# Anaesthesiaye/sound_event_detection_transformer

Measured on AMD Instinct MI355X. Metric: audio clips/sec training throughput (B=64, 10s@64-mel), higher is better.
Workload: dtype bf16; 1 GPU; URBAN-SED SEDT enc_layers=3 dec_at num_queries=10 B=64/GPU, 10 s @ 64-mel (B,1,500,64), full train step: fwd + Hungarian matching (device) + SetCriterion + bwd + clip 0.1 + AdamW, dropout 0.1; global_batch=64, parallelism=dp1

## Files before the change

sound_event_detection_transformer_amd/csrc/misc.hip:

```cpp
#include <stdarg.h>
#include <string.h>
#include <type_traits>
#include <algorithm>
#include "common.h"

namespace sedt {

static thread_local char g_err[512] = "";

void set_error(const char* fmt, ...) {
  va_list ap;
  va_start(ap, fmt);
  vsnprintf(g_err, sizeof(g_err), fmt, ap);
  va_end(ap);
}

int check_launch(const char* what) {
  hipError_t e = hipGetLastError();
  if (e != hipSuccess) {
    set_error("%s: launch failed: %s", what, hipGetErrorString(e));
    return 2;
  }
  return 0;
}

static inline hipStream_t S(void* s) { return reinterpret_cast<hipStream_t>(s); }
static inline unsigned nblk(long n, int per = 256) { return (unsigned)((n + per - 1) / per); }


struct ReduceJobs {
  int n;
  SedtReduceJob j[SEDT_MAX_REDUCE_JOBS];
  const uint32_t* pf[3]; int pf_lines[3];
};

__host__ __device__ inline int reduce_job_mode(const SedtReduceJob& J) {
  if ((reinterpret_cast<uintptr_t>(J.slab) | reinterpret_cast<uintptr_t>(J.out)) & 15) return 2;
  if (J.taps == 1 && (J.Ci & 3) == 0) return J.splitk >= 16 ? 3 : 0;
  if (J.taps > 1 && J.taps <= 9 && (J.Ci & 63) == 0) return 1;
  return 2;
}
__host__ __device__ inline int reduce_job_blocks(const SedtReduceJob& J) {
  const long per = (long)J.R * J.taps * J.Ci;
  const int mode = reduce_job_mode(J);
  if (mode == 0) return (int)((per + 1023) / 1024);
  if (mode == 1) return J.R * (J.Ci / 64);
  return (int)((per + 255) / 256);
}

__global__ __launch_bounds__(256) void multi_wgrad_reduce_kernel(const ReduceJobs jobs) {
  __shared__ float tile[9][65];
  if (blockIdx.x < 256 && jobs.pf_lines[0] + jobs.pf_lines[1] + jobs.pf_lines[2] > 0) {
    const int slot = blockIdx.x >> 3, nslots = min(32, max(1, (int)(gridDim.x >> 3)));
    uint32_t acc = 0;
    for (int r = 0; r < 3; ++r)
      for (int j = slot * 256 + threadIdx.x; j < jobs.pf_lines[r]; j += nslots * 256) acc ^= jobs.pf[r][(long)j * 32];
    if (acc == 0x9e3779b9u && jobs.n < 0) tile[0][0] = 1.f;
  }
  int lo = 0, hi = jobs.n - 1;
  while (lo < hi) {
    int mid = (lo + hi + 1) >> 1;
    if (jobs.j[mid].blk0 <= (int)blockIdx.x) lo = mid; else hi = mid - 1;
  }
  const SedtReduceJob& J = jobs.j[lo];
  const int blk = blockIdx.x - J.blk0;
  const long per = (long)J.R * J.taps * J.Ci;
  if (J.colsum_slab) {
    __shared__ float csum[4][64];
    const int col = blk * 64 + (threadIdx.x & 63), zg = threadIdx.x >> 6;
    if (blk * 64 < J.R) {
      float b0 = 0.f, b1 = 0.f, b2 = 0.f, b3 = 0.f;
      if (col < J.R) {
        const float* cp = J.colsum_slab + col;
        const int csk = J.cs_splitk > 0 ? J.cs_splitk : J.splitk;
        int z = zg;
        for (; z + 12 < csk; z += 16) {
          b0 += cp[(long)z * J.R];
          b1 += cp[(long)(z + 4) * J.R];
          b2 += cp[(long)(z + 8) * J.R];
          b3 += cp[(long)(z + 12) * J.R];
        }
        for (; z < csk; z += 4) b0 += cp[(long)z * J.R];
      }
      csum[zg][threadIdx.x & 63] = (b0 + b1) + (b2 + b3);
      __syncthreads();
      if (zg == 0 && col < J.R) J.bias_out[col] = (csum[0][col & 63] + csum[1][col & 63]) + (csum[2][col & 63] + csum[3][col & 63]);
    }
  }
  const int mode = reduce_job_mode(J);
  if (mode == 3) {
    __shared__ float4 zsum[4][64];
    const int q = threadIdx.x & 63, zg = threadIdx.x >> 6;
    const long e = ((long)blk * 64 + q) * 4;
    float4 s0 = make_float4(0.f, 0.f, 0.f, 0.f), s1 = s0;
    if (e < per) {
      const float* sp = J.slab + e;
      int z = zg;
      for (; z + 4 < J.splitk; z += 8) {
        const float4 a = *reinterpret_cast<const float4*>(sp + (long)z * per);
        const float4 b = *reinterpret_cast<const float4*>(sp + (long)(z + 4) * per);
        s0.x += a.x; s0.y += a.y; s0.z += a.z; s0.w += a.w;
        s1.x += b.x; s1.y += b.y; s1.z += b.z; s1.w += b.w;
      }
      if (z < J.splitk) {
        const float4 a = *reinterpret_cast<const float4*>(sp + (long)z * per);
        s0.x += a.x; s0.y += a.y; s0.z += a.z; s0.w += a.w;
      }
    }
    zsum[zg][q] = make_float4(s0.x + s1.x, s0.y + s1.y, s0.z + s1.z, s0.w + s1.w);
    __syncthreads();
    if (zg == 0 && e < per) {
      const float4 a = zsum[0][q], b = zsum[1][q], c = zsum[2][q], d = zsum[3][q];
      float4 s = make_float4((a.x + b.x) + (c.x + d.x), (a.y + b.y) + (c.y + d.y), (a.z + b.z) + (c.z + d.z), (a.w + b.w) + (c.w + d.w));
      if (J.rowscale) {
        const float sc = J.rowscale[e / J.Ci];
        s.x *= sc; s.y *= sc; s.z *= sc; s.w *= sc;
      }
      *reinterpret_cast<float4*>(J.out + e) = s;
    }
  } else if (mode == 0) {
    const long e = ((long)blk * 256 + threadIdx.x) * 4;
    if (e >= per) return;
    const float* sp = J.slab + e;
    float4 s0 = *reinterpret_cast<const float4*>(sp), s1 = make_float4(0.f, 0.f, 0.f, 0.f), s2 = s1, s3 = s1;
    int z = 1;
    for (; z + 4 <= J.splitk; z += 4) {
      const float4 a = *reinterpret_cast<const float4*>(sp + (long)z * per);
      const float4 b = *reinterpret_cast<const float4*>(sp + (long)(z + 1) * per);
      const float4 c = *reinterpret_cast<const float4*>(sp + (long)(z + 2) * per);
      const float4 d = *reinterpret_cast<const float4*>(sp + (long)(z + 3) * per);
      s0.x += a.x; s0.y += a.y; s0.z += a.z; s0.w += a.w;
      s1.x += b.x; s1.y += b.y; s1.z += b.z; s1.w += b.w;
      s2.x += c.x; s2.y += c.y; s2.z += c.z; s2.w += c.w;
      s3.x += d.x; s3.y += d.y; s3.z += d.z; s3.w += d.w;
    }
    for (; z < J.splitk; ++z) {
      const float4 a = *reinterpret_cast<const float4*>(sp + (long)z * per);
      s0.x += a.x; s0.y += a.y; s0.z += a.z; s0.w += a.w;
    }
    float4 s = make_float4((s0.x + s1.x) + (s2.x + s3.x), (s0.y + s1.y) + (s2.y + s3.y), (s0.z + s1.z) + (s2.z + s3.z),
                           (s0.w + s1.w) + (s2.w + s3.w));
    if (J.rowscale) {
      const float sc = J.rowscale[e / J.Ci];
      s.x *= sc; s.y *= sc; s.z *= sc; s.w *= sc;
    }
    *reinterpret_cast<float4*>(J.out + e) = s;
  } else if (mode == 1) {
    const int chunks = J.Ci / 64;
    const int r = blk / chunks, c0 = (blk - r * chunks) * 64;
    if (r >= J.R) return;
    const int n = J.taps * 64;
    const float sc = J.rowscale ? J.rowscale[r] : 1.f;
    const long rbase = (long)r * J.taps * J.Ci;
    for (int i = threadIdx.x; i < n / 4; i += 256) {
      const int tap = i >> 4, c = (i & 15) * 4;
      const float* sp = J.slab + rbase + (long)tap * J.Ci + c0 + c;
      float4 v = *reinterpret_cast<const float4*>(sp), u = make_float4(0.f, 0.f, 0.f, 0.f);
      int z = 1;
      for (; z + 2 <= J.splitk; z += 2) {
        const float4 a = *reinterpret_cast<const float4*>(sp + (long)z * per);
        const float4 b = *reinterpret_cast<const float4*>(sp + (long)(z + 1) * per);
        v.x += a.x; v.y += a.y; v.z += a.z; v.w += a.w;
        u.x += b.x; u.y += b.y; u.z += b.z; u.w += b.w;
      }
      if (z < J.splitk) {
        const float4 a = *reinterpret_cast<const float4*>(sp + (long)z * per);
        v.x += a.x; v.y += a.y; v.z += a.z; v.w += a.w;
      }
      tile[tap][c] = (v.x + u.x) * sc; tile[tap][c + 1] = (v.y + u.y) * sc;
      tile[tap][c + 2] = (v.z + u.z) * sc; tile[tap][c + 3] = (v.w + u.w) * sc;
    }
    __syncthreads();
    float* o = J.out + ((long)r * J.Ci + c0) * J.taps;
    if (J.taps == 9) {
      for (int i = threadIdx.x; i < n / 4; i += 256) {
        float4 q;
        { const int k = 4 * i, c = k / 9, tap = k - c * 9; q.x = tile[tap][c]; }
        { const int k = 4 * i + 1, c = k / 9, tap = k - c * 9; q.y = tile[tap][c]; }
        { const int k = 4 * i + 2, c = k / 9, tap = k - c * 9; q.z = tile[tap][c]; }
        { const int k = 4 * i + 3, c = k / 9, tap = k - c * 9; q.w = tile[tap][c]; }
        *reinterpret_cast<float4*>(o + 4 * i) = q;
      }
    } else {
      for (int i = threadIdx.x; i < n; i += 256) {
        const int c = i / J.taps, tap = i - c * J.taps;
        o[i] = tile[tap][c];
      }
    }
  } else {
    const long e = (long)blk * 256 + threadIdx.x;
    if (e >= per) return;
    const int c = (int)(e % J.Ci);
    const long rt = e / J.Ci;
    const int tap = (int)(rt % J.taps);
    const int r = (int)(rt / J.taps);
    float s = 0.f;
    for (int z = 0; z < J.splitk; ++z) s += J.slab[(long)z * per + e];
    if (J.rowscale) s *= J.rowscale[r];
    J.out[((long)r * J.Ci + c) * J.taps + tap] = s;
  }
}

template <typename TI>
__global__ void colsum_kernel(const TI* __restrict__ in, long ld, int rows, int cols, int rows_per_chunk,
                              float* __restrict__ out) {
  __shared__ float red[4][64];
  int tx = threadIdx.x & 63, ty = threadIdx.x >> 6;
  int col = blockIdx.x * 64 + tx;
  int r0 = blockIdx.y * rows_per_chunk, r1 = min(rows, r0 + rows_per_chunk);
  float s = 0.f;
  if (col < cols)
    for (int r = r0 + ty; r < r1; r += 4) s += (float)in[(long)r * ld + col];
  red[ty][tx] = s;
  __syncthreads();
  if (ty == 0 && col < cols) out[(long)blockIdx.y * cols + col] = red[0][tx] + red[1][tx] + red[2][tx] + red[3][tx];
}

static int colsum_chunks(int rows) {
  int c = (rows + 255) / 256;
  return c < 1 ? 1 : (c > 256 ? 256 : c);
}

template <typename T>
__global__ void dropout_grad_kernel(const T* __restrict__ in, long ldi, T* __restrict__ out, long ldo, int rows, int cols,
                                    uint32_t thresh, float inv_keep, uint32_t seed, const uint32_t* seed_ptr) {
  long e = (long)blockIdx.x * blockDim.x + threadIdx.x;
  if (e >= (long)rows * cols) return;
  int r = (int)(e / cols), c = (int)(e % cols);
  uint32_t sd = eff_seed(seed, seed_ptr);
  float v = (float)in[(long)r * ldi + c];
  out[(long)r * ldo + c] = (T)(drop_keep(sd, (uint64_t)e, thresh) ? v * inv_keep : 0.f);
}

template <typename T>
__global__ void add_kernel(const T* __restrict__ a, const T* __restrict__ b, T* __restrict__ out, int rows, int cols,
                           int b_mod) {
  long e = (long)blockIdx.x * blockDim.x + threadIdx.x;
  if (e >= (long)rows * cols) return;
  int r = (int)(e / cols), c = (int)(e % cols);
  int rb = b_mod > 0 ? r % b_mod : r;
  out[e] = (T)((float)a[e] + (float)b[(long)rb * cols + c]);
}

struct AddN { const void* p[8]; int n; };
template <typename T>
__global__ void add_n_kernel(const AddN a, T* __restrict__ out, long n8) {
  const long e = (long)blockIdx.x * blockDim.x + threadIdx.x;
  if (e >= n8) return;
  float acc[8];
#pragma unroll
  for (int i = 0; i < 8; ++i) acc[i] = 0.f;
  for (int j = 0; j < a.n; ++j) {
    const VecT<T, 8> v = reinterpret_cast<const VecT<T, 8>*>(a.p[j])[e];
#pragma unroll
    for (int i = 0; i < 8; ++i) acc[i] += (float)v.v[i];
  }
  VecT<T, 8> o;
#pragma unroll
  for (int i = 0; i < 8; ++i) o.v[i] = (T)acc[i];
  reinterpret_cast<VecT<T, 8>*>(out)[e] = o;
}

template <typename TI, typename TO>
__global__ void cast_kernel(const TI* __restrict__ in, TO* __restrict__ out, long n) {
  long e = (long)blockIdx.x * blockDim.x + threadIdx.x;
  if (e < n) out[e] = (TO)(float)in[e];
}

template <typename T>
__global__ void relu_mask_kernel(const T* __restrict__ g, const T* __restrict__ y, T* __restrict__ out, long n) {
  long e = (long)blockIdx.x * blockDim.x + threadIdx.x;
  if (e < n) out[e] = ((float)y[e] > 0.f) ? g[e] : (T)0.f;
}

template <typename T>
__global__ void gelu_fwd_kernel(const T* __restrict__ h, T* __restrict__ a, long n8, uint32_t thresh, float inv_keep, uint32_t seed,
                                const uint32_t* seed_ptr) {
  const long e = (long)blockIdx.x * blockDim.x + threadIdx.x;
  if (e >= n8) return;
  const uint32_t sd = eff_seed(seed, seed_ptr);
  const VecT<T, 8> v = reinterpret_cast<const VecT<T, 8>*>(h)[e];
  VecT<T, 8> o;
#pragma unroll
  for (int i = 0; i < 8; ++i) {
    const float x = (float)v.v[i];
    const float y = 0.5f * x * (1.f + erff(x * 0.70710678118654752f));
    o.v[i] = (T)((thresh == 0u || drop_keep(sd, (uint64_t)(e * 8 + i), thresh)) ? y * inv_keep : 0.f);
  }
  reinterpret_cast<VecT<T, 8>*>(a)[e] = o;
}

template <typename T>
__global__ void gelu_bwd_kernel(const T* __restrict__ g, const T* __restrict__ h, T* __restrict__ out, long n8, uint32_t thresh,
                                float inv_keep, uint32_t seed, const uint32_t* seed_ptr) {
  const long e = (long)blockIdx.x * blockDim.x + threadIdx.x;
  if (e >= n8) return;
  const uint32_t sd = eff_seed(seed, seed_ptr);
  const VecT<T, 8> gv = reinterpret_cast<const VecT<T, 8>*>(g)[e];
  const VecT<T, 8> hv = reinterpret_cast<const VecT<T, 8>*>(h)[e];
  VecT<T, 8> o;
#pragma unroll
  for (int i = 0; i < 8; ++i) {
    const float x = (float)hv.v[i];
    const float d = 0.5f * (1.f + erff(x * 0.70710678118654752f)) + x * 0.39894228040143268f * expf(-0.5f * x * x);
    o.v[i] = (T)((thresh == 0u || drop_keep(sd, (uint64_t)(e * 8 + i), thresh)) ? (float)gv.v[i] * d * inv_keep : 0.f);
  }
  reinterpret_cast<VecT<T, 8>*>(out)[e] = o;
}

__global__ void sigmoid_grad_kernel(const float* g, const float* s, float* out, long n) {
  long e = (long)blockIdx.x * blockDim.x + threadIdx.x;
  if (e < n) out[e] = g[e] * s[e] * (1.f - s[e]);
}

constexpr int COPY_MAXJ = 8;
struct CopyJobs {
  int n;
  SedtCopyJob j[COPY_MAXJ];
};
__global__ __launch_bounds__(256) void copy2d_kernel(const CopyJobs jobs) {
  int i = 0;
  while (i + 1 < jobs.n && (int)blockIdx.x >= jobs.j[i + 1].blk0) ++i;
  const SedtCopyJob& J = jobs.j[i];
  const long w = (long)(blockIdx.x - J.blk0) * 256 + threadIdx.x;
  const long per = J.inner / 4;
  if (w >= per * J.outer) return;
  const long o = w / per, k = w - o * per;
  reinterpret_cast<uint32_t*>(reinterpret_cast<char*>(J.dst) + o * J.dst_stride)[k] =
      reinterpret_cast<const uint32_t*>(reinterpret_cast<const char*>(J.src) + o * J.src_stride)[k];
}

template <typename T>
__global__ void spsedt_dec_in_kernel(const T* __restrict__ patch, const float* __restrict__ query, const float* __restrict__ keep_in,
                                     float* __restrict__ keep_out, T* __restrict__ out, int B, int Q, int P, int qpp, int D, int train,
                                     uint32_t thresh, uint32_t seed, const uint32_t* seed_ptr) {
  const int row = blockIdx.x * (blockDim.x / 32) + threadIdx.x / 32;
  if (row >= B * Q) return;
  const int b = row / Q, q = row - b * Q, c0 = (threadIdx.x & 31) * 8;
  float k = 1.f;
  if (train) {
    if (keep_in) k = keep_in[(long)q * B + b];
    else k = (thresh == 0u || drop_keep(eff_seed(seed, seed_ptr), (uint64_t)q * B + b, thresh)) ? 1.f : 0.f;
    if (keep_out && c0 == 0) keep_out[(long)q * B + b] = k;
  }
  const float qs = train ? 2.f : 1.f;
  for (int c = c0; c < D; c += 256) {
    const VecT<T, 8> pv = *reinterpret_cast<const VecT<T, 8>*>(patch + ((long)b * P + q / qpp) * D + c);
    const float4 qa = *reinterpret_cast<const float4*>(query + (long)q * D + c), qb = *reinterpret_cast<const float4*>(query + (long)q * D + c + 4);
    const float qv[8] = {qa.x, qa.y, qa.z, qa.w, qb.x, qb.y, qb.z, qb.w};
    VecT<T, 8> o;
#pragma unroll
    for (int i = 0; i < 8; ++i) o.v[i] = (T)(qs * qv[i] + k * (float)pv.v[i]);
    *reinterpret_cast<VecT<T, 8>*>(out + (long)row * D + c) = o;
  }
}

template <typename T>
__global__ void spsedt_dec_in_bwd_kernel(const T* __restrict__ g, const float* __restrict__ keep, T* __restrict__ d_patch,
                                         float* __restrict__ d_query, int B, int Q, int P, int qpp, int D, int train) {
  __shared__ float part[3][1024 / 4];
  const int blk = blockIdx.x;
  const int c = threadIdx.x % D, grp = threadIdx.x / D;
  if (blk < B * P) {
    if (!d_patch || grp) return;
    const int b = blk / P, p = blk - b * P;
    float acc = 0.f;
    for (int r = 0; r < qpp; ++r) {
      const int q = p * qpp + r;
      if (q >= Q) break;
      const float k = (train && keep) ? keep[(long)q * B + b] : 1.f;
      acc += k * (float)g[((long)b * Q + q) * D + c];
    }
    d_patch[(long)blk * D + c] = (T)acc;
    return;
  }
  const int q = blk - B * P;
  const int per = (B + 3) / 4, b0 = grp * per, b1 = min(B, b0 + per);
  float acc = 0.f;
  int b = b0;
  for (; b + 8 <= b1; b += 8) {
    float v[8];
#pragma unroll
    for (int i = 0; i < 8; ++i) v[i] = (float)g[((long)(b + i) * Q + q) * D + c];
#pragma unroll
    for (int i = 0; i < 8; ++i) acc += v[i];
  }
  for (; b < b1; ++b) acc += (float)g[((long)b * Q + q) * D + c];
  if (grp) part[grp - 1][c] = acc;
  __syncthreads();
  if (!grp) d_query[(long)q * D + c] = (train ? 2.f : 1.f) * (((acc + part[0][c]) + part[1][c]) + part[2][c]);
}

__global__ void bn_fold_kernel(const float* w, const float* b, const float* rm, const float* rv, float* scale,
                               float* bias, int n) {
  int i = blockIdx.x * blockDim.x + threadIdx.x;
  if (i >= n) return;
  float sc = w[i] * rsqrtf(rv[i] + 1e-5f);
  scale[i] = sc;
  bias[i] = b[i] - rm[i] * sc;
}

template <typename T>
__global__ void pack_conv_kernel(const float* __restrict__ w, int Cout, int Cin, int taps, const float* bnscale,
                                 T* __restrict__ wf, T* __restrict__ wb) {
  long e = (long)blockIdx.x * blockDim.x + threadIdx.x;
  long n = (long)Cout * Cin * taps;
  if (e >= n) return;
  int tap = (int)(e % taps);
  long r = e / taps;
  int ci = (int)(r % Cin), co = (int)(r / Cin);
  float v = w[e];
  if (wf) wf[((long)co * taps + tap) * Cin + ci] = (T)v;
  if (wb) wb[((long)ci * taps + tap) * Cout + co] = (T)(bnscale ? v * bnscale[co] : v);
}

template <typename T>
__global__ void stem_prep_kernel(const float* w0, const float* b0, const float* w1, T* wcat) {
  int e = blockIdx.x * blockDim.x + threadIdx.x;
  if (e >= 64 * 128) return;
  int co = e >> 7, k = e & 127;
  float v = 0.f;
  int tap = k & 63;
  if (tap < 49) {
    const float* src = (k < 64) ? w0 : b0;
    for (int c = 0; c < 3; ++c) v += w1[(co * 3 + c) * 49 + tap] * src[c];
  }
  wcat[e] = (T)v;
}

template <typename T>
__global__ __launch_bounds__(256) void stem_im2col_kernel(const float* __restrict__ x, T* __restrict__ col, int B, int H, int W,
                                                          int Ho, int Wo) {
  extern __shared__ float rows[];
  const int P = W + 6;
  const int ho = blockIdx.y, b = blockIdx.z;
  const float* xb = x + (long)b * H * W;
  for (int i = threadIdx.x; i < 7 * P; i += 256) {
    const int kh = i / P, j = i - kh * P;
    const int hi = 2 * ho - 3 + kh, wi = j - 3;
    rows[i] = ((unsigned)hi < (unsigned)H && (unsigned)wi < (unsigned)W) ? xb[hi * W + wi] : 0.f;
  }
  __syncthreads();
  const int wo = blockIdx.x * 16 + (threadIdx.x >> 4), chunk = threadIdx.x & 15;
  if (wo >= Wo) return;
  const int pix = (b * Ho + ho) * Wo + wo;
  const int k0 = chunk * 8;
  const bool ind = k0 >= 64;
  VecT<T, 8> out;
#pragma unroll
  for (int e = 0; e < 8; ++e) {
    const int tap = (k0 & 63) + e;
    float v = 0.f;
    if (tap < 49) {
      const int kh = tap / 7, kw = tap - kh * 7;
      const int hi = 2 * ho - 3 + kh, wi = 2 * wo - 3 + kw;
      if (ind) v = ((unsigned)hi < (unsigned)H && (unsigned)wi < (unsigned)W) ? 1.f : 0.f;
      else v = rows[kh * P + 2 * wo + kw];
    }
    out.v[e] = (T)v;
  }
  *reinterpret_cast<VecT<T, 8>*>(col + (long)pix * 128 + k0) = out;
}

__global__ void stem_conv0_grad_kernel(const float* G, const float* w1, float* dw0, float* db0) {
  __shared__ float red[6][256];
  int t = threadIdx.x;
  float acc[6] = {0, 0, 0, 0, 0, 0};
  for (int e = t; e < 64 * 49; e += 256) {
    int co = e / 49, tap = e - co * 49;
    float gx = G[co * 128 + tap], gb = G[co * 128 + 64 + tap];
    for (int c = 0; c < 3; ++c) {
      float w = w1[(co * 3 + c) * 49 + tap];
      acc[c] += w * gx;
      acc[3 + c] += w * gb;
    }
  }
  for (int i = 0; i < 6; ++i) red[i][t] = acc[i];
  __syncthreads();
  for (int s = 128; s > 0; s >>= 1) {
    if (t < s)
      for (int i = 0; i < 6; ++i) red[i][t] += red[i][t + s];
    __syncthreads();
  }
  if (t < 3) dw0[t] = red[t][0];
  else if (t < 6) db0[t - 3] = red[t][0];
}

template <typename T, int VEC>
__global__ __launch_bounds__(256) void maxpool_fwd_kernel(const T* __restrict__ x, T* __restrict__ y, uint8_t* __restrict__ idx,
// ... 970 lines not shown
```

sound_event_detection_transformer_amd/functional.py:

```python
from collections import namedtuple

import torch
from torch.autograd import Function

from . import ops, packing, runtime
from .lib import F32, BF16
from .ops import ACT_NONE, ACT_RELU, ACT_SIGMOID, ConvGeom


def _dt_of(t):
    return F32 if t.dtype == torch.float32 else BF16


def _as(t, dt):
    want = torch.float32 if dt == F32 else torch.bfloat16
    t = t.contiguous()
    return t if t.dtype == want else ops.cast(t, dt)


def _wf(dt, w):
    return w if dt == F32 else ops.cast(w, BF16)


def _wb(dt, w):
    return ops.pack_conv(dt, w, want_fwd=False)[1]


def _prep_linear(dt, w, need_b):
    hit = packing.lookup(w)
    if hit is not None:
        return hit[0], hit[1]
    return _wf(dt, w), (_wb(dt, w) if need_b else None)


def _prep_conv(dt, w, bn):
    hit = packing.lookup(w)
    if hit is not None and hit[2] is not None:
        return hit
    sc, bi = ops.bn_fold(bn[0], bn[1], bn[2], bn[3])
    wf, wb = ops.pack_conv(dt, w, bnscale=sc)
    return wf, wb, sc, bi


class LinearFn(Function):

    @staticmethod
    def forward(ctx, x, weight, bias, act, out_f32, dt, relu_input=False, x_bits=None):
        x = _as(x, dt)
        ctx.relu_input = relu_input
        ctx.x_bits = x_bits if relu_input else None
        ctx.dt, ctx.act, ctx.out_f32 = dt, act, out_f32
        ctx.has_bias = bias is not None
        ctx.skinny = ops.skinny_ok(weight.shape[0], weight.shape[1]) and out_f32 and weight.is_contiguous()
        if ctx.skinny:
            y = ops.skinny_linear_fwd(dt, x, weight, bias, act, True)
            ctx.save_for_backward(x, weight, y if act != ACT_NONE else None)
            return y
        wf, ctx.wb = _prep_linear(dt, weight, ctx.needs_input_grad[0])
        y = ops.linear(dt, x, wf, bias=bias, act=act, out_f32=out_f32)
        ctx.save_for_backward(x, weight, y if act != ACT_NONE else None)
        return y

    @staticmethod
    def backward(ctx, gy):
        x, weight, y = ctx.saved_tensors
        dt = ctx.dt
        gy = gy.contiguous()
        if ctx.skinny:
            gx, gw, gb = ops.skinny_linear_bwd(dt, gy.float() if gy.dtype != torch.float32 else gy, y, weight, x, ctx.act,
                                               mask=x if ctx.relu_input else None, need_gx=ctx.needs_input_grad[0],
                                               need_gw=ctx.needs_input_grad[1], need_gb=ctx.has_bias and ctx.needs_input_grad[2])
            return gx, gw, gb, None, None, None, None, None
        if ctx.act == ACT_SIGMOID:
            gy = ops.sigmoid_grad(gy.float() if gy.dtype != torch.float32 else gy, y.float() if y.dtype != torch.float32 else y)
        elif ctx.act == ACT_RELU:
            gy = ops.relu_mask(_dt_of(gy), gy, y)
        g = _as(gy, dt)
        gx = None
        if ctx.needs_input_grad[0]:
            if ctx.relu_input and ctx.x_bits is not None:
                gx = ops.linear(dt, g, ctx.wb, mask=ctx.x_bits, ldm=ctx.x_bits.stride(0), mask_bits=True)
            else:
                gx = ops.linear(dt, g, ctx.wb, mask=x, ldm=x.stride(0)) if ctx.relu_input else ops.linear(dt, g, ctx.wb)
        gb = torch.empty((g.shape[1],), device=g.device, dtype=torch.float32) if (ctx.has_bias and ctx.needs_input_grad[2]) else None
        if ctx.needs_input_grad[1]:
            gw = ops.linear_wgrad(dt, g, x, bias_out=gb)
        else:
            gw = None
            if gb is not None:
                ops.colsum(dt, g, out=gb)
        return gx, gw, gb, None, None, None, None, None


class PoolAtFn(Function):

    @staticmethod
    def forward(ctx, logits, boxes, attn, mode, q0, Q):
        f32c = lambda t: t.detach() if (t.dtype == torch.float32 and t.is_contiguous()) else t.detach().float().contiguous()
        lg = f32c(logits)
        bx = f32c(boxes) if mode == 'weighted_sum' else None
        at = f32c(attn) if mode == 'attn' else None
        ctx.cfg = (mode, q0, Q)
        ctx.dts = (logits.dtype, None if boxes is None else boxes.dtype, None if attn is None else attn.dtype)
        ctx.save_for_backward(lg, bx, at)
        return ops.pool_at(lg, bx, at, mode, q0, Q)

    @staticmethod
    def backward(ctx, g):
        lg, bx, at = ctx.saved_tensors
        mode, q0, Q = ctx.cfg
        gl, gb, ga = ops.pool_at_bwd(lg, bx, at, mode, q0, Q, g)
        return (gl.to(ctx.dts[0]), None if gb is None else gb.to(ctx.dts[1]), None if ga is None else ga.to(ctx.dts[2]),
                None, None, None)


class HeadsFn(Function):

    @staticmethod
    def forward(ctx, hs, wc, bc, w1, b1, w2, b2, w3, b3, wa, ba, dt):
        Lh, B, Qp, d = hs.shape
        x = _as(hs, dt).view(Lh * B * Qp, d)
        tr = any(ctx.needs_input_grad)
        ctx.slab = None
        if ops.heads_slab_ok(dt, d, wc.shape[0], 0 if wa is None else wa.shape[0], hs.numel() // d) and wc.is_contiguous() and w3.is_contiguous():
            fr = [packing.lookup_frag(w) for w in (w1, w2)]
            if all(f is not None for f in fr):
                cls, box, at, hh = ops.heads_fwd(x, wc, bc, fr[0][0], b1, fr[1][0], b2, w3, b3, wa, ba, Lh, B, Qp, train=tr)
                ctx.dt, ctx.dims, ctx.has_at = dt, (Lh, B, Qp, d), wa is not None
                if tr:
                    ctx.slab = (fr[0][1], fr[1][1])
                    ctx.save_for_backward(x, hh[0], hh[1], box, at, wc, w3, wa)
                cls, box = cls.view(Lh, B, Qp, -1), box.view(Lh, B, Qp, 2)
                return (cls, box, at) if at is not None else (cls, box)
        cls = ops.skinny_linear_fwd(dt, x, wc, bc, ACT_NONE, True)
        w1f, w1b = _prep_linear(dt, w1, tr)
        w2f, w2b = _prep_linear(dt, w2, tr)
        h1 = ops.linear(dt, x, w1f, bias=b1, act=ACT_RELU)
        h2 = ops.linear(dt, h1, w2f, bias=b2, act=ACT_RELU)
        box = ops.skinny_linear_fwd(dt, h2, w3, b3, ACT_SIGMOID, True)
        at = None
        if wa is not None:
            xa = x.view(Lh, B, Qp, d)[Lh - 1, :, 0, :]
            at = ops.skinny_linear_fwd(dt, xa, wa, ba, ACT_SIGMOID, True)
        ctx.dt, ctx.dims, ctx.wb = dt, (Lh, B, Qp, d), (w1b, w2b)
        ctx.has_at = wa is not None
        ctx.save_for_backward(x, h1, h2, box, at, wc, w3, wa)
        cls, box = cls.view(Lh, B, Qp, -1), box.view(Lh, B, Qp, 2)
        return (cls, box, at) if at is not None else (cls, box)

    @staticmethod
    def backward(ctx, g_cls, g_box, g_at=None):
        x, h1, h2, box, at, wc, w3, wa = ctx.saved_tensors
        dt = ctx.dt
        Lh, B, Qp, d = ctx.dims
        M = Lh * B * Qp
        if ctx.slab is not None:
            f32c = lambda t: None if t is None else (t.contiguous() if t.dtype == torch.float32 else t.contiguous().float())
            C1, CA = wc.shape[0], 0 if wa is None else wa.shape[0]
            w1t, w2t = ctx.slab
            dhs, g_h1, g_h2, part = ops.heads_bwd(x, h1, h2, box.view(M, 2), at, f32c(g_cls).view(M, -1), f32c(g_box).view(M, 2),
                                                  f32c(g_at) if ctx.has_at else None, wc, w3, wa, w2t, w1t, Lh, B, Qp)
            rb = ops.ReduceBatch()
            d_b2 = torch.empty((d,), device=x.device, dtype=torch.float32)
            d_w2 = ops.linear_wgrad(dt, g_h2, h1, bias_out=d_b2, batch=rb)
            d_b1 = torch.empty((d,), device=x.device, dtype=torch.float32)
            d_w1 = ops.linear_wgrad(dt, g_h1, x, bias_out=d_b1, batch=rb)
            NG = C1 + CA + 2
            tot = torch.empty((NG * 257,), device=x.device, dtype=torch.float32)
            rb.add_colsum(part, part.shape[0], NG * 257, tot)
            rb.flush()
            tw, tb = tot[:NG * 256].view(NG, 256), tot[NG * 256:]
            d_wc, d_bc = tw[:C1], tb[:C1]
            d_w3, d_b3 = tw[C1 + CA:], tb[C1 + CA:]
            d_wa = d_ba = None
            if ctx.has_at:
                d_wa, d_ba = tw[C1:C1 + CA], tb[C1:C1 + CA]
            return (dhs.view(Lh, B, Qp, d), d_wc, d_bc, d_w1, d_b1, d_w2, d_b2, d_w3, d_b3, d_wa, d_ba, None)
        w1b, w2b = ctx.wb
        f32 = lambda t: t.contiguous() if t.dtype == torch.float32 else t.contiguous().float()
        rb = ops.ReduceBatch()
        dhs, d_wc, d_bc = ops.skinny_linear_bwd(dt, f32(g_cls).view(M, -1), None, wc, x, ACT_NONE, batch=rb)
        g_h2, d_w3, d_b3 = ops.skinny_linear_bwd(dt, f32(g_box).view(M, 2), box.view(M, 2), w3, h2, ACT_SIGMOID, mask=h2, batch=rb)
        d_b2 = torch.empty((g_h2.shape[1],), device=x.device, dtype=torch.float32)
        d_w2 = ops.linear_wgrad(dt, g_h2, h1, bias_out=d_b2, batch=rb)
        g_h1 = ops.linear(dt, g_h2, w2b, mask=h1, ldm=h1.stride(0))
        d_b1 = torch.empty((g_h1.shape[1],), device=x.device, dtype=torch.float32)
        d_w1 = ops.linear_wgrad(dt, g_h1, x, bias_out=d_b1, batch=rb)
        dhs = ops.linear(dt, g_h1, w1b, res=dhs, ldr=dhs.stride(0))
        d_wa = d_ba = None
        if ctx.has_at:
            xa = x.view(Lh, B, Qp, d)[Lh - 1, :, 0, :]
            if g_at is None:
                d_wa, d_ba = torch.zeros_like(wa), torch.zeros(wa.shape[0], device=wa.device)
            else:
                ga = f32(g_at).view(B, -1)
                _, d_wa, d_ba = ops.skinny_linear_bwd(dt, ga, at.view(B, -1), wa, xa, ACT_SIGMOID,
                                                      gx_acc=dhs.view(Lh, B, Qp, d)[Lh - 1, :, 0, :], batch=rb)
        rb.flush()
        return (dhs.view(Lh, B, Qp, d), d_wc, d_bc, d_w1, d_b1, d_w2, d_b2, d_w3, d_b3, d_wa, d_ba, None)


class SplitClipsFn(Function):

    @staticmethod
    def forward(ctx, n, dims, *ts):
        ctx.set_materialize_grads(False)
        ts = [t.contiguous() for t in ts]
        metas, outs_a, outs_b, jobs = [], [], [], []
        for t, d in zip(ts, dims):
            B = t.shape[d]
            outer = 1
            for s_ in t.shape[:d]:
                outer *= s_
            per = t.numel() // (outer * B) * t.element_size()
            a = torch.empty(t.shape[:d] + (n,) + t.shape[d + 1:], device=t.device, dtype=t.dtype)
            b = torch.empty(t.shape[:d] + (B - n,) + t.shape[d + 1:], device=t.device, dtype=t.dtype)
            jobs.append((t.data_ptr(), a.data_ptr(), outer, n * per, B * per, n * per))
            jobs.append((t.data_ptr() + n * per, b.data_ptr(), outer, (B - n) * per, B * per, (B - n) * per))
            metas.append((tuple(t.shape), t.dtype, outer, per, B))
            outs_a.append(a)
            outs_b.append(b)
        ops.copy2d(jobs)
        ctx.n, ctx.metas = n, metas
        return tuple(outs_a + outs_b)

    @staticmethod
    def backward(ctx, *gs):
        k = len(ctx.metas)
        grads, jobs = [], []
        for i, (shape, dtype, outer, per, B) in enumerate(ctx.metas):
            ga, gb = gs[i], gs[k + i]
            if ga is None and gb is None:
                grads.append(None)
                continue
            n = ctx.n
            full = torch.empty(shape, device=(ga if ga is not None else gb).device, dtype=dtype)
            if ga is None or gb is None:
                full.zero_()
            if ga is not None:
                ga = ga.contiguous().to(dtype)
                jobs.append((ga.data_ptr(), full.data_ptr(), outer, n * per, n * per, B * per))
            if gb is not None:
                gb = gb.contiguous().to(dtype)
                jobs.append((gb.data_ptr(), full.data_ptr() + n * per, outer, (B - n) * per, (B - n) * per, B * per))
            grads.append(full)
            ctx.keep = getattr(ctx, 'keep', []) + [ga, gb]
        if jobs:
            ops.copy2d(jobs)
        ctx.keep = None
        return (None, None) + tuple(grads)


class FanoutFn(Function):

    @staticmethod
    def forward(ctx, x, n, dt):
        ctx.set_materialize_grads(False)
        ctx.dt = dt
        return tuple(x.view_as(x) for _ in range(n))

    @staticmethod
    def backward(ctx, *gs):
        gs = [_as(g, ctx.dt) for g in gs if g is not None]
        if not gs:
            return None, None, None
        if len(gs) == 1 or gs[0].numel() % 8:
            out = gs[0]
            for g in gs[1:]:
                out = out + g
            return out, None, None
        return ops.add_n(ctx.dt, gs), None, None


class SpDecInFn(Function):

    @staticmethod
    def forward(ctx, patch, query, keep, B, Q, P, qpp, train, ratio, dt):
        patch = _as(patch, dt)
        q = query.detach().float().contiguous()
        sp = runtime.seed_ptr(patch.device) if (train and keep is None and ratio > 0) else None
        out, keep_used = ops.spsedt_dec_in(dt, patch, q, B, Q, P, qpp, train, ratio, keep, runtime.next_seed() if sp is not None else 0, sp)
        ctx.cfg = (B, Q, P, qpp, train, dt, patch.dtype)
        ctx.save_for_backward(keep_used)
        return out

    @staticmethod
    def backward(ctx, g):
        B, Q, P, qpp, train, dt, _ = ctx.cfg
        keep, = ctx.saved_tensors
        d_patch, d_query = ops.spsedt_dec_in_bwd(dt, _as(g, dt), keep, B, Q, P, qpp, train, need_patch=ctx.needs_input_grad[0])
        return d_patch, d_query, None, None, None, None, None, None, None, None


class GradAccumulator(object):

    def __init__(self, n_nodes):
        self.n, self.seen, self.pending, self.parts = n_nodes, 0, None, []

    def last(self):
        self.seen += 1
        done = self.seen == self.n
        if done:
            self.seen = 0
        return done

    def take_parts(self):
        p, self.parts = self.parts, []
        return p

    def take_pending(self):
        p, self.pending = self.pending, None
        return p


class LayerNormFn(Function):
    @staticmethod
    def forward(ctx, x, gamma, beta, dt):
        x = _as(x, dt)
        y, _, mean, rstd = ops.layernorm_fwd(dt, x, gamma, beta)
        ctx.dt = dt
        ctx.save_for_backward(x, gamma, mean, rstd)
        return y

    @staticmethod
    def backward(ctx, gy):
        x, gamma, mean, rstd = ctx.saved_tensors
        dx, dg, db = ops.layernorm_bwd(ctx.dt, _as(gy, ctx.dt), x, gamma, mean, rstd)
        return dx, dg, db, None


class StackViewFn(Function):

    @staticmethod
    def forward(ctx, buf, share, *outs):
        R = outs[0].shape[0]
        for i, o in enumerate(outs):
            if o.data_ptr() != buf.data_ptr() + i * R * buf.shape[1] * buf.element_size() or o.shape != outs[0].shape:
                raise RuntimeError('StackViewFn: the layer outputs are not the row ranges of the stacking buffer')
        ctx.R, ctx.n, ctx.share = R, len(outs), share
        return buf.view(buf.shape)

    @staticmethod
    def backward(ctx, g):
        g = g.contiguous()
        parts = [g[i * ctx.R:(i + 1) * ctx.R] for i in range(ctx.n)]
        if ctx.share is not None:
            ctx.share['stack_g'] = parts
            return (None, None) + (None,) * (ctx.n - 1) + (parts[-1],)
        return (None, None) + tuple(parts)


class BroadcastRowsFn(Function):

    @staticmethod
    def forward(ctx, table, zeros, B, dt):
        ctx.dt, ctx.B, ctx.shape = dt, B, tuple(table.shape)
        return ops.add(dt, zeros, _as(table.detach(), dt), table.shape[0])

    @staticmethod
    def backward(ctx, g):
        Q, C = ctx.shape
        g = _as(g, ctx.dt)
        return ops.colsum(ctx.dt, g.view(ctx.B, Q * C)).view(Q, C), None, None, None


class CastFn(Function):

    @staticmethod
    def forward(ctx, x, dt):
        ctx.src_dtype = x.dtype
        return _as(x, dt)

    @staticmethod
    def backward(ctx, g):
        return g.to(ctx.src_dtype), None


class AddFn(Function):

    @staticmethod
    def forward(ctx, a, b, b_mod, dt):
        ctx.set_materialize_grads(False)
        return ops.add(dt, _as(a, dt), _as(b, dt), b_mod)

    @staticmethod
    def backward(ctx, g):
        return g, None, None, None


def _mha_fwd(dt, q_in, k_in, v_in, same_qk, w_in, b_in, w_out, b_out, res, B, H, Lq, Lk, kpm, amask, p, seeds, train=True):
    E = w_in.shape[1]
    wf, wb_in = _prep_linear(dt, w_in, train)
    wf_o, wb_o = _prep_linear(dt, w_out, train)
    if same_qk:
        qk, v = ops.linear_group(dt, [(q_in, wf[:2 * E], dict(bias=b_in[:2 * E])), (v_in, wf[2 * E:], dict(bias=b_in[2 * E:]))])
        q, k = qk[:, :E], qk[:, E:]
    else:
        q, k, v = ops.linear_group(dt, [(q_in, wf[:E], dict(bias=b_in[:E])), (k_in, wf[E:2 * E], dict(bias=b_in[E:2 * E])),
                                        (v_in, wf[2 * E:], dict(bias=b_in[2 * E:]))])
        qk = None
    sp = runtime.seed_ptr(q_in.device) if p > 0 else None
    ctxv, lse = ops.attention_fwd(dt, q, k, v, B, H, Lq, Lk, kpm, amask, p, seeds[0], sp)
    out = ops.linear(dt, ctxv, wf_o, bias=b_out, drop_p=p, seed=seeds[1], seed_ptr=sp, res=res, ldr=res.stride(0))
    saved = dict(wb_in=wb_in, wb_o=wb_o, q_in=q_in, k_in=k_in, v_in=v_in, same_qk=same_qk, qk=qk, q=q, k=k, v=v, ctxv=ctxv, lse=lse,
                 dims=(B, H, Lq, Lk), kpm=kpm, amask=amask, p=p, seeds=seeds)
    return out, saved


def _drop_args(s, device):
    p = s['p']
    return (p, s['seeds'][1], runtime.seed_ptr(device) if p > 0 else None)


def _mha_bwd(dt, s, g_out, w_in, w_out, need_q=True, need_k=True, need_v=True, batch=None, g_dropped=None, kv_fused=False,
             res_kv=None):
    B, H, Lq, Lk = s['dims']
    E = w_in.shape[1]
    p = s['p']
    sp = runtime.seed_ptr(g_out.device) if p > 0 else None
    if g_dropped is not None:
        g1 = g_dropped
    else:
        g1 = ops.dropout_grad(dt, g_out, p, s['seeds'][1], sp) if p > 0 else g_out
    d_bo = torch.empty((E,), device=g_out.device, dtype=torch.float32)
    d_wo = ops.linear_wgrad(dt, g1, s['ctxv'], bias_out=d_bo, batch=batch, param=w_out)
    g_ctx = ops.linear(dt, g1, s['wb_o'])
    td = g_out.dtype
    if s['same_qk']:
        dqk = torch.empty((B * Lq, 2 * E), device=g_out.device, dtype=td)
        dq, dk = dqk[:, :E], dqk[:, E:]
        dv = torch.empty((B * Lk, E), device=g_out.device, dtype=td)
    elif kv_fused:
        dq = torch.empty((B * Lq, E), device=g_out.device, dtype=td)
        dkv = torch.empty((B * Lk, 2 * E), device=g_out.device, dtype=td)
        dk, dv = dkv[:, :E], dkv[:, E:]
    else:
        dq = torch.empty((B * Lq, E), device=g_out.device, dtype=td)
        dk = torch.empty((B * Lk, E), device=g_out.device, dtype=td)
        dv = torch.empty((B * Lk, E), device=g_out.device, dtype=td)
    ops.attention_bwd(dt, s['q'], s['k'], s['v'], s['ctxv'], g_ctx, s['lse'], B, H, Lq, Lk, dq, dk, dv, s['kpm'], s['amask'],
                      p, s['seeds'][0], sp)
    d_win = ops._sink(w_in, (3 * E, E))
    if d_win is None:
        d_win = torch.empty((3 * E, E), device=g_out.device, dtype=torch.float32)
    d_bin = torch.empty((3 * E,), device=g_out.device, dtype=torch.float32)
    wb = s['wb_in']
    g_q = g_k = g_v = None
    dgrads = []
    if s['same_qk']:
        ops.linear_wgrad(dt, dqk, s['q_in'], out=d_win[:2 * E], bias_out=d_bin[:2 * E], batch=batch)
        if need_q or need_k:
            dgrads.append(('q', dqk, wb[:, :2 * E]))
    else:
        ops.linear_wgrad(dt, dq, s['q_in'], out=d_win[:E], bias_out=d_bin[:E], batch=batch)
        ops.linear_wgrad(dt, dk, s['k_in'], out=d_win[E:2 * E], bias_out=d_bin[E:2 * E], batch=batch)
        if need_q:
            dgrads.append(('q', dq, wb[:, :E]))
        if need_k and not kv_fused:
            dgrads.append(('k', dk, wb[:, E:2 * E]))
    ops.linear_wgrad(dt, dv, s['v_in'], out=d_win[2 * E:], bias_out=d_bin[2 * E:], batch=batch)
    if kv_fused and not s['same_qk']:
        dgrads.append(('v', dkv, wb[:, E:], {} if res_kv is None else dict(res=res_kv, ldr=res_kv.stride(0))))
    elif need_v:
        dgrads.append(('v', dv, wb[:, 2 * E:]))
    if dgrads:
        got = dict(zip([d[0] for d in dgrads], ops.linear_group(dt, [(d[1], d[2], dict(d[3]) if len(d) > 3 else {}) for d in dgrads])))
        g_q, g_k, g_v = got.get('q'), got.get('k'), got.get('v')
    return g_q, g_k, g_v, d_win, d_bin, d_wo, d_bo


def _ffn_fwd(dt, x_in, w1, b1, w2, b2, res, p, seeds, train=True, out=None, act='relu'):
    sp = runtime.seed_ptr(x_in.device) if p > 0 else None
    wf1, wb1 = _prep_linear(dt, w1, train)
    wf2, wb2 = _prep_linear(dt, w2, train)
    if act == 'gelu':
        h_pre = ops.linear(dt, x_in, wf1, bias=b1)
        h = ops.gelu_fwd(dt, h_pre, p, seeds[0], sp)
        out = ops.linear(dt, h, wf2, out, bias=b2, drop_p=p, seed=seeds[1], seed_ptr=sp, res=res, ldr=res.stride(0))
        return out, dict(x_in=x_in, h=h, h_pre=h_pre, p=p, seeds=seeds, wb1=wb1, wb2=wb2)
    h = ops.linear(dt, x_in, wf1, bias=b1, act=ACT_RELU, drop_p=p, seed=seeds[0], seed_ptr=sp)
    out = ops.linear(dt, h, wf2, out, bias=b2, drop_p=p, seed=seeds[1], seed_ptr=sp, res=res, ldr=res.stride(0))
    return out, dict(x_in=x_in, h=h, p=p, seeds=seeds, wb1=wb1, wb2=wb2)


def _ffn_bwd(dt, s, g_out, w1, w2, res_for_gx=None, batch=None, g_dropped=None):
    p = s['p']
    if g_dropped is not None:
        g2 = g_dropped
    else:
        g2 = ops.dropout_grad(dt, g_out, p, s['seeds'][1], runtime.seed_ptr(g_out.device)) if p > 0 else g_out
    d_b2 = torch.empty((g2.shape[1],), device=g2.device, dtype=torch.float32)
    d_w2 = ops.linear_wgrad(dt, g2, s['h'], bias_out=d_b2, batch=batch, param=w2)
    if s.get('h_pre') is not None:
        gh = ops.gelu_bwd(dt, ops.linear(dt, g2, s['wb2']), s['h_pre'], p, s['seeds'][0], runtime.seed_ptr(g2.device) if p > 0 else None)
    else:
        gh = ops.linear(dt, g2, s['wb2'], mask=s['h'], ldm=s['h'].stride(0), alpha=1.0 / (1.0 - p) if p > 0 else 1.0)
    d_b1 = torch.empty((gh.shape[1],), device=gh.device, dtype=torch.float32)
    d_w1 = ops.linear_wgrad(dt, gh, s['x_in'], bias_out=d_b1, batch=batch, param=w1)
    if res_for_gx is not None:
        gx = ops.linear(dt, gh, s['wb1'], res=res_for_gx, ldr=res_for_gx.stride(0))
    else:
        gx = ops.linear(dt, gh, s['wb1'])
    return gx, d_w1, d_b1, d_w2, d_b2


class EncoderLayerFn(Function):

    @staticmethod
    def forward(ctx, x, pos, kpm, amask, cfg, *P):
        dt = cfg['dt']
        (w_in, b_in, w_o, b_o, w1, b1, w2, b2, g1, be1, g2, be2) = P
        B, S, H = cfg['B'], cfg['S'], cfg['H']
        p = cfg['dropout'] if cfg['training'] else 0.0
        seeds = [runtime.next_seed() for _ in range(4)]
        x = _as(x, dt)
        pos = _as(pos, dt)
        sv = {}
        tr = any(ctx.needs_input_grad)
        fr = None
        act = cfg.get('act', 'relu')
        if cfg['pre_norm'] and act == 'relu' and ops.encoder_slab_ok(dt, x.shape[1], H, S, w1.shape[0], amask, B):
            fr = [packing.lookup_frag(w) for w in (w_in, w_o, w1, w2)]
            fr = fr if all(f is not None for f in fr) else None
        if fr is not None:
            x, pos = x.contiguous(), pos.contiguous()
            sp = runtime.seed_ptr(x.device) if p > 0 else None
            _, wb_in = _prep_linear(dt, w_in, tr)
            _, wb_o = _prep_linear(dt, w_o, tr)
            _, wb1 = _prep_linear(dt, w1, tr)
            _, wb2 = _prep_linear(dt, w2, tr)
            qk, v, by1 = ops.encoder_qkv_fwd(x, pos, g1, be1, fr[0][0], b_in, B, S, train=tr, prefetch=(fr[1][0], fr[2][0], fr[3][0]))
            x2, by2 = ops.encoder_attn_ffn_fwd(x, qk, v, kpm, fr[1][0], b_o, g2, be2, fr[2][0], b1, fr[3][0], b2, B, S, w1.shape[0],
                                               p, seeds, sp, train=tr)
            if tr:
                xn, xnp, m1, r1 = by1
                ctxv, lse, x1, m2, r2, x1n, h = by2
                E = x.shape[1]
                sv['mha'] = dict(wb_in=wb_in, wb_o=wb_o, q_in=xnp, k_in=xnp, v_in=xn, same_qk=True, qk=qk, q=qk[:, :E], k=qk[:, E:], v=v,
                                 ctxv=ctxv, lse=lse, dims=(B, H, S, S), kpm=kpm, amask=None, p=p, seeds=seeds[0:2])
                sv['ffn'] = dict(x_in=x1n, h=h, p=p, seeds=seeds[2:4], wb1=wb1, wb2=wb2)
                sv.update(x=x, x1=x1, m1=m1, r1=r1, m2=m2, r2=r2, slab=(fr[0][1], fr[1][1], fr[2][1], fr[3][1]))
                chain = cfg.get('chain')
                if chain is not None:
                    sv['bwd_next'], chain.top = chain.top, (fr[3][1], fr[2][1], fr[1][1])
            ctx.sv, ctx.cfg, ctx.P = sv, cfg, P
            return x2
        if cfg['pre_norm']:
            xn, xnp, m1, r1 = ops.layernorm_fwd(dt, x, g1, be1, add_t=pos)
            x1, sv['mha'] = _mha_fwd(dt, xnp, xnp, xn, True, w_in, b_in, w_o, b_o, x, B, H, S, S, kpm, amask, p, seeds[0:2], tr)
            x1n, _, m2, r2 = ops.layernorm_fwd(dt, x1, g2, be2)
            x2, sv['ffn'] = _ffn_fwd(dt, x1n, w1, b1, w2, b2, x1, p, seeds[2:4], tr, act=act)
            sv.update(x=x, x1=x1, m1=m1, r1=r1, m2=m2, r2=r2)
        else:
            xp = ops.add(dt, x, pos)
            t, sv['mha'] = _mha_fwd(dt, xp, xp, x, True, w_in, b_in, w_o, b_o, x, B, H, S, S, kpm, amask, p, seeds[0:2], tr)
            x1, _, m1, r1 = ops.layernorm_fwd(dt, t, g1, be1)
            t2, sv['ffn'] = _ffn_fwd(dt, x1, w1, b1, w2, b2, x1, p, seeds[2:4], tr, act=act)
            x2, _, m2, r2 = ops.layernorm_fwd(dt, t2, g2, be2)
            sv.update(t=t, t2=t2, m1=m1, r1=r1, m2=m2, r2=r2)
        ctx.sv, ctx.cfg, ctx.P = sv, cfg, P
        return x2

    @staticmethod
    def backward(ctx, gx2):
        sv, cfg, P = ctx.sv, ctx.cfg, ctx.P
        dt = cfg['dt']
        (w_in, b_in, w_o, b_o, w1, b1, w2, b2, g1, be1, g2, be2) = P
        gx2 = _as(gx2, dt)
        share = cfg.get('wg_share') if not (sv.get('slab') is not None and ops.SLAB_ENC_BWD) else None
        rb = share.batch() if share is not None else ops.ReduceBatch()
        if sv.get('slab') is not None and ops.SLAB_ENC_BWD:
            B, S, H = cfg['B'], cfg['S'], cfg['H']
            wint, wot, w1t, w2t = sv['slab']
            ff, mh = sv['ffn'], sv['mha']
            p = ff['p']
            dev = gx2.device
            sp = runtime.seed_ptr(dev) if p > 0 else None
            E = gx2.shape[1]
            g2d, gh, gx1, g1d, gctx, part2 = ops.encoder_ffn_bwd(gx2.contiguous(), ff['h'], sv['x1'], sv['m2'], sv['r2'], g2, w2t, w1t, wot,
                                                                 B, S, p, (ff['seeds'][1], mh['seeds'][1]), sp)
            d_b2 = torch.empty((E,), device=dev, dtype=torch.float32)
            d_w2 = ops.linear_wgrad(dt, g2d, ff['h'], bias_out=d_b2, batch=rb, param=w2)
            d_b1 = torch.empty((gh.shape[1],), device=dev, dtype=torch.float32)
            d_w1 = ops.linear_wgrad(dt, gh, ff['x_in'], bias_out=d_b1, batch=rb, param=w1)
            d_bo = torch.empty((E,), device=dev, dtype=torch.float32)
            d_wo = ops.linear_wgrad(dt, g1d, mh['ctxv'], bias_out=d_bo, batch=rb, param=w_o)
            dgb2 = torch.empty((2 * E,), device=dev, dtype=torch.float32)
            rb.add_colsum(part2, part2.shape[0], 2 * E, dgb2)
            dqk = torch.empty((B * S, 2 * E), device=dev, dtype=gx2.dtype)
            dv = torch.empty((B * S, E), device=dev, dtype=gx2.dtype)
            ops.attention_bwd(dt, mh['q'], mh['k'], mh['v'], mh['ctxv'], gctx, mh['lse'], B, H, S, S, dqk[:, :E], dqk[:, E:], dv, mh['kpm'],
                              None, p, mh['seeds'][0], sp)
            d_win = ops._sink(w_in, (3 * E, E))
            if d_win is None:
                d_win = torch.empty((3 * E, E), device=dev, dtype=torch.float32)
            d_bin = torch.empty((3 * E,), device=dev, dtype=torch.float32)
            ops.linear_wgrad(dt, dqk, mh['q_in'], out=d_win[:2 * E], bias_out=d_bin[:2 * E], batch=rb)
            ops.linear_wgrad(dt, dv, mh['v_in'], out=d_win[2 * E:], bias_out=d_bin[2 * E:], batch=rb)
            gx, part1 = ops.encoder_qkv_bwd(dqk, dv, sv['x'], sv['m1'], sv['r1'], g1, gx1, wint, B, S)
            dgb1 = torch.empty((2 * E,), device=dev, dtype=torch.float32)
            rb.add_colsum(part1, part1.shape[0], 2 * E, dgb1)
            rb.flush(prefetch=sv.get('bwd_next'))
            ctx.sv = None
            return (gx, None, None, None, None, d_win, d_bin, d_wo, d_bo, d_w1, d_b1, d_w2, d_b2, dgb1[:E], dgb1[E:], dgb2[:E], dgb2[E:])
        if cfg['pre_norm']:
            g_x1n, d_w1, d_b1, d_w2, d_b2 = _ffn_bwd(dt, sv['ffn'], gx2, w1, w2, batch=rb)
            gx1, d_g2, d_be2, gx1d = ops.layernorm_bwd(dt, g_x1n, sv['x1'], g2, sv['m2'], sv['r2'], dres=gx2, batch=rb,
                                                       drop=_drop_args(sv['mha'], gx2.device))
            g_qk, _, g_v, d_win, d_bin, d_wo, d_bo = _mha_bwd(dt, sv['mha'], gx1, w_in, w_o, batch=rb, g_dropped=gx1d)
            gx, d_g1, d_be1 = ops.layernorm_bwd(dt, g_v, sv['x'], g1, sv['m1'], sv['r1'], dy2=g_qk, dres=gx1, batch=rb)
        else:
            dev = gx2.device
            g_t2, d_g2, d_be2, g_t2d = ops.layernorm_bwd(dt, gx2, sv['t2'], g2, sv['m2'], sv['r2'], batch=rb,
                                                         drop=_drop_args(sv['ffn'], dev))
            g_x1, d_w1, d_b1, d_w2, d_b2 = _ffn_bwd(dt, sv['ffn'], g_t2, w1, w2, res_for_gx=g_t2, batch=rb, g_dropped=g_t2d)
            g_t, d_g1, d_be1, g_td = ops.layernorm_bwd(dt, g_x1, sv['t'], g1, sv['m1'], sv['r1'], batch=rb,
                                                       drop=_drop_args(sv['mha'], dev))
            g_qk, _, g_v, d_win, d_bin, d_wo, d_bo = _mha_bwd(dt, sv['mha'], g_t, w_in, w_o, batch=rb, g_dropped=g_td)
            gx = ops.add(dt, ops.add(dt, g_qk, g_v), g_t)
        if share is not None:
            share.layer_done(last=cfg.get('layer_idx', 0) == 0)
        else:
            rb.flush()
        ctx.sv = None
        return (gx, None, None, None, None, d_win, d_bin, d_wo, d_bo, d_w1, d_b1, d_w2, d_b2, d_g1, d_be1, d_g2, d_be2)


class DecoderLayerFn(Function):

    @staticmethod
    def forward(ctx, tgt, mem, mem_pos, qpos, kpm, tgt_mask, cfg, *P):
        dt = cfg['dt']
        (sw_in, sb_in, sw_o, sb_o, cw_in, cb_in, cw_o, cb_o, w1, b1, w2, b2, g1, be1, g2, be2, g3, be3) = P
        B, S, Q, H = cfg['B'], cfg['S'], cfg['Q'], cfg['H']
        p = cfg['dropout'] if cfg['training'] else 0.0
        seeds = [runtime.next_seed() for _ in range(6)]
        tgt, mem, mem_pos, qpos = _as(tgt, dt), _as(mem, dt), _as(mem_pos, dt), _as(qpos, dt)
        sv = {}
        tr = any(ctx.needs_input_grad)
        if cfg['pre_norm']:
            tn, tnp, m1, r1 = ops.layernorm_fwd(dt, tgt, g1, be1, add_t=qpos)
            t1, sv['sa'] = _mha_fwd(dt, tnp, tnp, tn, True, sw_in, sb_in, sw_o, sb_o, tgt, B, H, Q, Q, None, tgt_mask, p, seeds[0:2], tr)
            t1n, t1np, m2, r2 = ops.layernorm_fwd(dt, t1, g2, be2, add_t=qpos)
            t2, sv['ca'] = _mha_fwd(dt, t1np, mem_pos, mem, False, cw_in, cb_in, cw_o, cb_o, t1, B, H, Q, S, kpm, None, p, seeds[2:4], tr)
            t2n, _, m3, r3 = ops.layernorm_fwd(dt, t2, g3, be3)
            t3, sv['ffn'] = _ffn_fwd(dt, t2n, w1, b1, w2, b2, t2, p, seeds[4:6], tr, out=cfg.get('out'), act=cfg.get('act', 'relu'))
            sv.update(tgt=tgt, t1=t1, t2=t2, m1=m1, r1=r1, m2=m2, r2=r2, m3=m3, r3=r3)
        else:
            tp = ops.add(dt, tgt, qpos)
            a, sv['sa'] = _mha_fwd(dt, tp, tp, tgt, True, sw_in, sb_in, sw_o, sb_o, tgt, B, H, Q, Q, None, tgt_mask, p, seeds[0:2], tr)
            t1, _, m1, r1 = ops.layernorm_fwd(dt, a, g1, be1)
            t1p = ops.add(dt, t1, qpos)
            c, sv['ca'] = _mha_fwd(dt, t1p, mem_pos, mem, False, cw_in, cb_in, cw_o, cb_o, t1, B, H, Q, S, kpm, None, p, seeds[2:4], tr)
            t2, _, m2, r2 = ops.layernorm_fwd(dt, c, g2, be2)
            f, sv['ffn'] = _ffn_fwd(dt, t2, w1, b1, w2, b2, t2, p, seeds[4:6], tr, act=cfg.get('act', 'relu'))
            t3, _, m3, r3 = ops.layernorm_fwd(dt, f, g3, be3)
            sv.update(a=a, c=c, f=f, m1=m1, r1=r1, m2=m2, r2=r2, m3=m3, r3=r3)
        if tr and cfg.get('chain') is not None and cfg.get('layer_idx', 0) == 0:
            sv['bwd_next'] = cfg['chain'].top
        ctx.sv, ctx.cfg, ctx.P = sv, cfg, P
        return t3

    @staticmethod
    def backward(ctx, g3_):
        sv, cfg, P = ctx.sv, ctx.cfg, ctx.P
        dt = cfg['dt']
        (sw_in, sb_in, sw_o, sb_o, cw_in, cb_in, cw_o, cb_o, w1, b1, w2, b2, g1, be1, g2, be2, g3, be3) = P
        gt3 = _as(g3_, dt)
        share = cfg.get('wg_share')
        rb = share.batch() if share is not None else ops.ReduceBatch()
        if cfg['pre_norm']:
            g_t2n, d_w1, d_b1, d_w2, d_b2 = _ffn_bwd(dt, sv['ffn'], gt3, w1, w2, batch=rb)
            gt2, d_g3, d_be3, gt2d = ops.layernorm_bwd(dt, g_t2n, sv['t2'], g3, sv['m3'], sv['r3'], dres=gt3, batch=rb,
                                                       drop=_drop_args(sv['ca'], gt3.device))
            kvf = cfg.get('kv_fused', False)
            acc_m = cfg.get('acc_mem') if kvf else None
            acc_q = cfg.get('acc_qpos')
            g_q, g_k, g_v, d_cwin, d_cbin, d_cwo, d_cbo = _mha_bwd(dt, sv['ca'], gt2, cw_in, cw_o, batch=rb, g_dropped=gt2d, kv_fused=kvf,
                                                                   res_kv=None if acc_m is None else acc_m.take_pending())
            gt1, d_g2, d_be2, gt1d = ops.layernorm_bwd(dt, g_q, sv['t1'], g2, sv['m2'], sv['r2'], dres=gt2, batch=rb,
                                                       drop=_drop_args(sv['sa'], gt3.device))
            g_qpos = g_q
            g_mem_pos, g_mem = g_k, g_v
            g_qk, _, g_vs, d_swin, d_sbin, d_swo, d_sbo = _mha_bwd(dt, sv['sa'], gt1, sw_in, sw_o, batch=rb, g_dropped=gt1d)
            sg = cfg.get('share', {}).get('stack_g') if cfg.get('share') is not None else None
            extra = sg[cfg['layer_idx'] - 1] if (sg is not None and cfg.get('layer_idx', 0) > 0) else None
            gtgt, d_g1, d_be1 = ops.layernorm_bwd(dt, g_vs, sv['tgt'], g1, sv['m1'], sv['r1'], dy2=g_qk, dres=gt1, batch=rb, dres2=extra)
            if acc_m is not None and not acc_m.last():
                acc_m.pending, g_mem = g_mem, None
            if acc_q is not None:
                acc_q.parts += [g_q, g_qk]
                g_qpos = ops.add_n(dt, acc_q.take_parts()) if acc_q.last() else None
            else:
                g_qpos = ops.add(dt, g_qpos, g_qk)
        else:
            dev = gt3.device
            g_f, d_g3, d_be3, g_fd = ops.layernorm_bwd(dt, gt3, sv['f'], g3, sv['m3'], sv['r3'], batch=rb,
                                                       drop=_drop_args(sv['ffn'], dev))
            g_t2, d_w1, d_b1, d_w2, d_b2 = _ffn_bwd(dt, sv['ffn'], g_f, w1, w2, res_for_gx=g_f, batch=rb, g_dropped=g_fd)
            g_c, d_g2, d_be2, g_cd = ops.layernorm_bwd(dt, g_t2, sv['c'], g2, sv['m2'], sv['r2'], batch=rb,
                                                       drop=_drop_args(sv['ca'], dev))
            g_q, g_k, g_v, d_cwin, d_cbin, d_cwo, d_cbo = _mha_bwd(dt, sv['ca'], g_c, cw_in, cw_o, batch=rb, g_dropped=g_cd,
                                                                   kv_fused=cfg.get('kv_fused', False))
            g_t1 = ops.add(dt, g_q, g_c)
            g_qpos = g_q
            g_mem_pos, g_mem = g_k, g_v
            g_a, d_g1, d_be1, g_ad = ops.layernorm_bwd(dt, g_t1, sv['a'], g1, sv['m1'], sv['r1'], batch=rb,
                                                       drop=_drop_args(sv['sa'], dev))
            g_qk, _, g_vs, d_swin, d_sbin, d_swo, d_sbo = _mha_bwd(dt, sv['sa'], g_a, sw_in, sw_o, batch=rb, g_dropped=g_ad)
            gtgt = ops.add(dt, ops.add(dt, g_qk, g_vs), g_a)
            g_qpos = ops.add(dt, g_qpos, g_qk)
        if share is not None:
            share.layer_done(last=cfg.get('layer_idx', 0) == 0, prefetch=sv.get('bwd_next'))
        else:
            rb.flush(prefetch=sv.get('bwd_next'))
        ctx.sv = None
        return (gtgt, g_mem, g_mem_pos, g_qpos, None, None, None,
                d_swin, d_sbin, d_swo, d_sbo, d_cwin, d_cbin, d_cwo, d_cbo, d_w1, d_b1, d_w2, d_b2,
                d_g1, d_be1, d_g2, d_be2, d_g3, d_be3)


def _bn(bn):
    return ops.bn_fold(bn[0], bn[1], bn[2], bn[3])


class StemFn(Function):

    @staticmethod
    def forward(ctx, x, w0, b0, w1, bnw, bnb, bnrm, bnrv, dt):
        B, _, H, W = x.shape
        x = x.contiguous().float()
        wcat = ops.stem_prep(dt, w0, b0, w1)
        _, _, sc, bi = _prep_conv(dt, w1, (bnw, bnb, bnrm, bnrv))
        ctx.direct = ops.stem_pool_ok(dt, W)
        if ctx.direct:
            pool, idx, Hp, Wp = ops.stem_pool_fwd(x, wcat, sc, bi, B, H, W, want_idx=any(ctx.needs_input_grad))
            ctx.dt, ctx.dims = dt, (B, H, W)
            if idx is not None:
                ctx.save_for_backward(x, pool, idx, sc, w1)
            ctx.out_hw = (Hp, Wp)
            return pool
        col, Ho, Wo = ops.stem_im2col(dt, x, B, H, W)
        s1 = ops.linear(dt, col, wcat, scale=sc, bias=bi, act=ACT_RELU)
        pool, idx, Hp, Wp = ops.maxpool_fwd(dt, s1, B, Ho, Wo, 64)
        ctx.dt, ctx.dims = dt, (B, Ho, Wo)
        ctx.save_for_backward(col, pool, idx, sc, w1)
        ctx.mark_non_differentiable(idx)
        ctx.out_hw = (Hp, Wp)
        return pool

    @staticmethod
    def backward(ctx, g):
        col, pool, idx, sc, w1 = ctx.saved_tensors
        dt = ctx.dt
        if ctx.direct:
            B, H, W = ctx.dims
            G = ops.stem_pool_wgrad(col, _as(g, dt).contiguous(), idx, pool, sc, B, H, W)
            dw0, db0 = ops.stem_conv0_grad(G, w1)
            return None, dw0, db0, None, None, None, None, None, None
        B, Ho, Wo = ctx.dims
        gs = ops.maxpool_bwd(dt, _as(g, dt), idx, None, B, Ho, Wo, 64, y=pool)
        G = ops.wgrad(dt, gs, col, gs.shape[0], ConvGeom(1, 1, 128, 64), rowscale=sc).view(64, 128)
        dw0, db0 = ops.stem_conv0_grad(G, w1)
        return None, dw0, db0, None, None, None, None, None, None


class BlockCfg(object):
    __slots__ = ('cin', 'planes', 'stride', 'dil', 'ds')

    def __init__(self, cin, planes, stride, dil, ds):
        self.cin, self.planes, self.stride, self.dil, self.ds = cin, planes, stride, dil, ds


BlockPlan = namedtuple('BlockPlan', 'fwd want_ab want_bits mask_x bwd want_g want_gx wgrads')


def block_plan(dt, blk, B, H, W, first, mask_input, contiguous, have_xbits, train, need_x_grad, w_rg, have_frags, relu_bits):
    fwd = ops.block_form(dt, blk, W, B, H) if (contiguous and have_frags) else None
    row = ops.BLOCK_FORMS.get(fwd)
    trainable = any(w_rg)
    mask_x = (not first) or bool(mask_input)
    want_gx = (not first) or bool(need_x_grad)
    if not train or not (want_gx or trainable):
        bwd = 'skip'
    elif fwd == 'bneck0' and not trainable:
        bwd = 'chain'
    elif row is not None and row.nops == 3 and want_gx and (have_xbits or not mask_x):
        bwd = 'fused'
    else:
        bwd = 'per_op'
    if row is None:
        want_ab = True
    elif not row.ab_bits:
        want_ab = bool(train)
    else:
        want_ab = bool(train) and (trainable or (row.nops == 3 and mask_x and not have_xbits))
    assert bwd != 'per_op' or want_ab, (fwd, bwd)
    return BlockPlan(fwd, want_ab, bool(train and relu_bits), mask_x, bwd, bwd == 'fused' and trainable, want_gx,
                     tuple(bool(r) and bwd in ('fused', 'per_op') for r in w_rg))


class _BlockRec(object):
    __slots__ = ('plan', 'blk', 'x', 'a', 'b', 'y', 'xbits', 'H', 'W', 'geom', 's', 'wb', 'wt', 'ab_bits')

    def __init__(self, **kw):
        for k in self.__slots__:
            setattr(self, k, kw.get(k))


def _block_wgrads(dt, B, r, t, grads, base, batch, gp, gb=None, ga=None):
    def wg(k, g, act):
        if r.plan.wgrads[k]:
            grads[base + 5 * k] = ops.wgrad(dt, g, act, B, r.geom[k], rowscale=r.s[k], batch=batch, param=t[5 * k])
    wg(2, gp, r.b)
    if gb is None:
        gb = ops.conv_dgrad(dt, gp, B, r.geom[2], r.wb[2], mask=r.b, ldm=r.b.stride(0))
    wg(1, gb, r.a)
    if ga is None:
        ga = ops.conv_dgrad(dt, gb, B, r.geom[1], r.wb[1], mask=r.a, ldm=r.a.stride(0))
    wg(0, ga, r.x)
    if r.blk.ds:
        wg(3, gp, r.x)
    return ga


class StageFn(Function):

    @staticmethod
    def forward(ctx, x, meta, *T):
        dt, B, H, W, blocks = meta['dt'], meta['B'], meta['H'], meta['W'], meta['blocks']
        x = _as(x, dt)
        saved = []
        i = 0
        train = any(ctx.needs_input_grad)
        xbits = meta.get('x_bits')
        for bi_, blk in enumerate(blocks):
            n = 20 if blk.ds else 15
            t = T[i:i + n]
            i += n
            cin, pl = blk.cin, blk.planes
            prep = [_prep_conv(dt, t[k], t[k + 1:k + 5]) for k in range(0, n, 5)]
            g2 = ConvGeom(H, W, pl, pl, 3, blk.stride, blk.dil, blk.dil)
            geom = [ConvGeom(H, W, cin, pl, 1), g2, ConvGeom(g2.Ho, g2.Wo, pl, 4 * pl, 1)]
            if blk.ds:
                geom.append(ConvGeom(H, W, cin, 4 * pl, 1, blk.stride))
            cf = [packing.lookup_conv_frag(t[k]) for k in range(0, n, 5)]
            fragged = all(c is not None for c in cf)
            plan = block_plan(dt, blk, B, H, W, bi_ == 0, meta['mask_input'], x.is_contiguous(), xbits is not None, train,
                              ctx.needs_input_grad[0], [t[k].requires_grad for k in range(0, n, 5)], fragged, ops.RELU_BITS)
            rec = _BlockRec(plan=plan, blk=blk, x=x, xbits=xbits, H=H, W=W, geom=geom, s=[q[2] for q in prep], wb=[q[1] for q in prep])
            if plan.fwd is not None:
                nx = [packing.lookup_conv_frag(T[i + k]) for k in (0, 5, 10)] if (plan.fwd == 'bneck3' and i + 15 <= len(T)) else None
                nx = [c[0] for c in nx] if nx and all(c is not None for c in nx) else None
                y, rec.a, rec.b, ybits, *rec.ab_bits = ops.block_fwd(plan.fwd, x, B, H, W, [c[0] for c in cf], [(q[2], q[3]) for q in prep],
                                                                     train=train, want_bits=plan.want_bits, want_ab=plan.want_ab, nxt=nx)
                rec.wt = [c[1] for c in cf]
            else:
                (w1f, _, s1, b1), (w2f, _, s2, b2), (w3f, _, s3, b3) = prep[:3]
                rec.a = ops.conv_fwd(dt, x, B, geom[0], w1f, scale=s1, bias=b1, act=ACT_RELU)
                rec.b = ops.conv_fwd(dt, rec.a, B, g2, w2f, scale=s2, bias=b2, act=ACT_RELU)
                idn = ops.conv_fwd(dt, x, B, geom[3], prep[3][0], scale=prep[3][2], bias=prep[3][3]) if blk.ds else x
                g3 = geom[2]
                ybits = (torch.empty((B * g3.Ho * g3.Wo, g3.Co // 8), device=x.device, dtype=torch.uint8)
                         if (plan.want_bits and g3.Co % 8 == 0) else None)
                y = ops.conv_fwd(dt, rec.b, B, g3, w3f, scale=s3, bias=b3, res=idn, ldr=idn.stride(0), act=ACT_RELU, act_post_res=1,
                                 **({} if ybits is None else dict(bits_out=ybits)))
            rec.y = y
            saved.append(rec)
            x, H, W, xbits = y, g2.Ho, g2.Wo, ybits
        if meta.get('holder') is not None:
            meta['holder']['bits'] = xbits
        ctx.bwd_next = None
        chain = meta.get('chain')
        if train and ops.RELU_BITS and chain is not None:
            ctx.bwd_next = chain.top
            if saved and saved[-1].plan.fwd in ('bneck', 'bneck3'):
                chain.top = tuple(saved[-1].wt[:3])
        ctx.saved, ctx.meta, ctx.T = saved, meta, T
        ctx.out_hw = (H, W)
        return x

    @staticmethod
    def backward(ctx, gy):
        saved, meta, T = ctx.saved, ctx.meta, ctx.T
        dt, B = meta['dt'], meta['B']
        grads = [None] * len(T)
        gp = _as(gy, dt) if meta.get('grad_premasked') else ops.relu_mask(dt, _as(gy, dt), saved[-1].y)
        rb = ops.ReduceBatch()
        base = len(T)
        for bi_ in range(len(saved) - 1, -1, -1):
            r = saved[bi_]
            plan, g1, w1b = r.plan, r.geom[0], r.wb[0]
            n = 20 if r.blk.ds else 15
            base -= n
            t = T[base:base + n]
            if plan.bwd == 'skip':
                gp = None
                continue
            mask_by_x = dict(mask=r.x, ldm=r.x.stride(0)) if plan.mask_x else {}
            if plan.bwd == 'chain':
                _, _, ga = ops.bneck_bwd(gp, B, r.H, r.W, r.wt, *r.ab_bits, None, chain_only=True)
                side = ops.conv_dgrad(dt, gp, B, r.geom[3], r.wb[3])
                gp = ops.conv_dgrad(dt, ga, B, g1, w1b, res=side, ldr=side.stride(0), **mask_by_x)
                continue
            if plan.bwd == 'fused':
                prev = saved[bi_ - 1] if bi_ > 0 else None
                nx = prev.wt if (prev is not None and plan.fwd == 'bneck3' and prev.plan.fwd == 'bneck3') else None
                gx, gb, ga = ops.bneck_bwd(gp, B, r.H, r.W, r.wt, *r.ab_bits, r.xbits if plan.mask_x else None, want_g=plan.want_g, nxt=nx)
                if plan.want_g:
                    _block_wgrads(dt, B, r, t, grads, base, rb, gp, gb, ga)
                gp = gx
                continue
            ga = _block_wgrads(dt, B, r, t, grads, base, rb, gp)
            if plan.want_gx:
                side, ep_side = ops.proj_dgrad(dt, gp, B, r.geom[3], r.wb[3]) if r.blk.ds else (gp, dict(ldr=gp.stride(0)))
                if plan.mask_x and r.xbits is not None:
                    mask_by_x = dict(mask=r.xbits, ldm=r.xbits.stride(0), mask_bits=True)
                gp = ops.conv_dgrad(dt, ga, B, g1, w1b, res=side, **ep_side, **mask_by_x)
            else:
                gp = None
        rb.flush(prefetch=ctx.bwd_next)
        ctx.saved = None
        return (gp, None) + tuple(grads)
```

sound_event_detection_transformer_amd/ops.py:

```python
import ctypes as C
from collections import namedtuple

import os
import numpy as np
import torch

from . import lib as L
from .lib import F32, BF16, ACT_NONE, ACT_RELU, ACT_SIGMOID, TORCH_DTYPE, p as _p


class ConvGeom(object):
    __slots__ = ('Hi', 'Wi', 'Ci', 'Ho', 'Wo', 'Co', 'KH', 'KW', 'sh', 'sw', 'ph', 'pw', 'dh', 'dw')

    def __init__(self, Hi, Wi, Ci, Co, k=1, stride=1, pad=0, dil=1):
        self.Hi, self.Wi, self.Ci, self.Co = Hi, Wi, Ci, Co
        self.KH = self.KW = k
        self.sh = self.sw = stride
        self.ph = self.pw = pad
        self.dh = self.dw = dil
        self.Ho = (Hi + 2 * pad - dil * (k - 1) - 1) // stride + 1
        self.Wo = (Wi + 2 * pad - dil * (k - 1) - 1) // stride + 1

    @property
    def taps(self):
# ... 328 lines not shown
def linear(dtype, x, w, out=None, *, bias=None, out_f32=False, **ep):
    M, K = x.shape
    N = w.shape[0]
    if out is None:
        out = torch.empty((M, N), device=x.device, dtype=torch.float32 if out_f32 else TORCH_DTYPE[dtype])
    igemm(dtype, M, N, K, x, x.stride(0), w, w.stride(0), out, out.stride(0), bias=bias, out_f32=int(out_f32), **ep)
    return out


def skinny_ok(N, K):
    return N <= 16 and K % 64 == 0 and K <= 1024


def skinny_linear_fwd(dtype, x, w, bias=None, act=ACT_NONE, out_f32=False):
    _dev_check(x, w)
    M, K = x.shape
    N = w.shape[0]
    assert w.dtype == torch.float32 and w.is_contiguous() and x.stride(1) == 1
    y = torch.empty((M, N), device=x.device, dtype=torch.float32 if out_f32 else TORCH_DTYPE[dtype])
    L.check(L.load().sedt_skinny_linear_fwd(_p(x), x.stride(0), _p(w), _p(bias), _p(y), y.stride(0), M, N, K, act, int(out_f32), dtype,
                                            L.stream_ptr()), 'skinny_linear_fwd')
    return y


def skinny_linear_bwd(dtype, g, ysaved, w, x, act=ACT_NONE, mask=None, need_gx=True, need_gw=True, need_gb=True, gx_acc=None, batch=None):
    M, K = x.shape
    N = w.shape[0]
    assert g.dtype == torch.float32 and g.is_contiguous() and (ysaved is None or (ysaved.dtype == torch.float32 and ysaved.is_contiguous()))
    assert x.stride(1) == 1
    if gx_acc is not None:
        assert gx_acc.shape == (M, K) and gx_acc.stride(1) == 1 and gx_acc.dtype == TORCH_DTYPE[dtype] and mask is None
        gx = gx_acc
    else:
        gx = torch.empty((M, K), device=x.device, dtype=TORCH_DTYPE[dtype]) if need_gx else None
    dw = torch.empty((N, K), device=x.device, dtype=torch.float32) if need_gw else None
    db = torch.empty((N,), device=x.device, dtype=torch.float32) if (need_gb and need_gw) else None
    lib = L.load()
    scratch = torch.empty((lib.sedt_skinny_linear_bwd_scratch(K) // 4,), device=x.device, dtype=torch.float32) if need_gw else None
    deferred = need_gw and batch is not None
    L.check(lib.sedt_skinny_linear_bwd(_p(g), _p(ysaved), g.stride(0), _p(w), _p(x), x.stride(0), _p(mask),
                                       mask.stride(0) if mask is not None else 0, _p(gx), gx.stride(0) if gx is not None else K,
                                       None if deferred else _p(dw), None if deferred else _p(db),
                                       _p(scratch), M, N, K, act, int(gx_acc is not None), dtype, L.stream_ptr()), 'skinny_linear_bwd')
    if deferred:
        tot = torch.empty((17 * K,), device=x.device, dtype=torch.float32)
        batch.add_colsum(scratch, 16, 17 * K, tot)
        dw = tot[:N * K].view(N, K)
        db = tot[16 * K:16 * K + N] if need_gb else None
    if need_gb and not need_gw:
        db = g.sum(0) if act == ACT_NONE else (g * ysaved * (1 - ysaved)).sum(0) if act == ACT_SIGMOID else (g * (ysaved > 0)).sum(0)
    return gx, dw, db


def _group_label(jobs):
    return _describe((L.SedtIgemm * len(jobs))(*jobs), BF16, len(jobs)) or None


def linear_group(dtype, items):
    outs, args = [], []
    for x, w, kw in items:
        kw = dict(kw)
        M, K = x.shape
        N = w.shape[0]
        out_f32 = kw.pop('out_f32', False)
        out = kw.pop('out', None)
        if out is None:
            out = torch.empty((M, N), device=x.device, dtype=torch.float32 if out_f32 else TORCH_DTYPE[dtype])
        outs.append(out)
        args.append(((M, N, K, x, x.stride(0), w, w.stride(0), out, out.stride(0)), dict(out_f32=int(out_f32), **kw)))
    if len(args) == 1 or PROFILE is not None or (_co['on'] and POOL.gemms) or (dtype == F32 and L.GEMM_X3 and X3_FAST):
        hint = None
        if len(args) > 1 and PROFILE is not None and dtype == BF16:
            hint = ('group', _group_label([igemm_args(*a, **kw) for a, kw in args]), 1.0)
        for a, kw in args:
            igemm(dtype, *a, hint=hint, **kw)
        return outs
    arr = (L.SedtIgemm * len(args))(*[igemm_args(*a, **kw) for a, kw in args])
    L.check(L.load().sedt_igemm_group(arr, len(args), L.gemm_dtype(dtype), L.stream_ptr()), 'igemm_group')
    return outs


S2_PARITY = _dev_env('SEDT_S2_PARITY', '1') != '0'
DIL_HALVES = _dev_env('SEDT_DIL_HALVES', '1') != '0'


def _direct3x3_ok(kind, dtype, t, g, w, out, ep):
    return (CONV3_DIRECT and dtype == BF16 and g.Ci == 64 and g.Co == 64 and g.KH == 3 and g.KW == 3
            and g.sh == 1 and g.sw == 1 and g.ph == 1 and g.pw == 1 and g.dh == 1 and g.dw == 1 and g.Wi == 16
            and t.stride(0) == 64 and out.stride(0) == 64 and set(ep) <= {'scale', 'bias', 'act', 'mask', 'ldm', 'tile'}
            and ep.get('act', 0) in (0, ACT_RELU) and tuple(ep.get('tile', (0, 0))) == (0, 0)
            and (ep.get('mask') is None or (ep.get('ldm', 64) == 64 and ep.get('act', 0) == 0))
            and (kind == 'fwd' or ('scale' not in ep and 'bias' not in ep)))


def _grouped_ok(dtype, t, out, ep):
    x3 = dtype == F32 and L.GEMM_X3 and X3_FAST
    if _co['on'] or not (dtype == BF16 or x3):
        return False
    return not x3 or (t.dtype == torch.float32 and out.dtype == torch.float32 and t.data_ptr() % 16 == 0 and t.stride(0) % 4 == 0
                      and (ep.get('res') is None or ep['res'].dtype == torch.float32)
                      and (ep.get('mask') is None or ep.get('mask_bits') or ep['mask'].dtype == torch.float32))


def _s2_parity_ok(kind, dtype, dy, g, wb, out, ep):
    return (S2_PARITY and kind == 'dgrad' and _grouped_ok(dtype, dy, out, ep) and g.KH == 3 and g.KW == 3 and g.sh == 2 and g.sw == 2
            and g.ph == 1 and g.pw == 1 and g.dh == 1 and g.dw == 1 and g.Co % 64 == 0 and g.Ci % 8 == 0 and wb.stride(0) == 9 * g.Co
            and dy.stride(0) % 8 == 0 and out.stride(0) % 8 == 0 and set(ep) <= {'mask', 'ldm', 'mask_bits', 'res', 'ldr', 'alpha'})


def _dil_halves_ok(kind, dtype, t, g, w, out, ep):
    d = g.dh
    cin, cout = (g.Co, g.Ci) if kind == 'dgrad' else (g.Ci, g.Co)
    return (DIL_HALVES and _grouped_ok(dtype, t, out, ep) and g.KH == 3 and g.KW == 3 and g.sh == 1 and g.sw == 1 and g.dw == d and d >= 1
            and g.ph == d and g.pw == d and g.Wi == 2 * d and g.Wo == g.Wi and g.Ho == g.Hi and cin % 64 == 0 and cout % 128 == 0
            and w.stride(0) == 9 * cin and t.stride(0) % 8 == 0 and out.stride(0) % 8 == 0
            and set(ep) <= {'scale', 'bias', 'act', 'mask', 'ldm', 'mask_bits', 'res', 'ldr', 'alpha', 'bits_out', 'act_post_res'}
            and (t.shape[0] // 2 // 128) * (cout // 128) >= 96)


_FORMS = {'direct3x3': (_direct3x3_ok, 1.0), 's2_parity': (_s2_parity_ok, 0.25), 'dil_halves': (_dil_halves_ok, 2.0 / 3.0)}
CONV_FORMS = {'fwd': ('direct3x3', 'dil_halves'), 'dgrad': ('s2_parity', 'dil_halves', 'direct3x3')}


def conv_form(kind, dtype, t, g, w, out, ep):
    for form in CONV_FORMS[kind]:
        ok, share = _FORMS[form]
        if ok(kind, dtype, t, g, w, out, ep):
            return form, form != 'direct3x3' and dtype == F32, share
    return 'gemm', False, 1.0


def _s2_parity_subs(B, g, C_):
    for ph_ in (0, 1):
        nh, khs = (g.Hi + 1 - ph_) // 2, ([1] if ph_ == 0 else [0, 2])
        for pw_ in (0, 1):
            nw, kws = (g.Wi + 1 - pw_) // 2, ([1] if pw_ == 0 else [0, 2])
            if nh and nw:
                yield (B * nh * nw, (g.Ho, g.Wo, C_, nh, nw, len(khs), len(kws), 1, 1, ph_, pw_, 1, 1), (64, 64), (g.Hi, g.Wi, 2, 2, ph_, pw_),
                       [kh * 3 + kw for kh in khs for kw in kws])


def _dil_halves_subs(B, g, C_, transposed):
    d = g.dh
    for half in (0, 1):
        kw0 = (1 - half) if not transposed else half
        yield (B * g.Ho * d, (g.Hi, g.Wi, C_, g.Ho, d, 3, 2, 1, 1, d, (d if transposed else 0), d, d), (128, 128), (g.Ho, g.Wo, 1, 1, 0, half * d),
               [kh * 3 + kw0 + j for kh in range(3) for j in range(2)])


def conv_group_jobs(form, kind, t, B, g, w, out, ep, x3):
    transposed = kind == 'dgrad'
    cin, cout = (g.Co, g.Ci) if transposed else (g.Ci, g.Co)
    C_ = cin
    if x3:
        t, w = _split3([(t, 0, B * (g.Ho * g.Wo if transposed else g.Hi * g.Wi), cin, t.stride(0), 0), (w, 0, cout * 9, cin, cin, 1)])
        w = w.view(cout, 27 * cin)
        C_ = 3 * cin
    jobs = []
    for M, conv, tile, omap, taps in (_s2_parity_subs(B, g, C_) if form == 's2_parity' else _dil_halves_subs(B, g, C_, transposed)):
        a = igemm_args(M, cout, len(taps) * C_, t, t.stride(0), w, w.stride(0), out, out.stride(0), conv=conv, transposed=int(transposed),
                       tile=tile, out_f32=int(x3), **ep)
        a.omap, (a.o_Hi, a.o_Wi, a.o_sh, a.o_sw, a.o_h0, a.o_w0) = 1, omap
        a.btap_on, a.f32ep, a.awrap = 1, int(x3), (cin if x3 else 0)
        for i, tap in enumerate(taps):
            a.btap[i] = tap * C_
        jobs.append(a)
    return jobs


def conv_hint(kind, plan, t, B, g, w, out, ep):
    form, x3, share = plan
    if form == 'direct3x3':
        return 'conv3x3_c64_kernel'
    if form == 'gemm' or x3:
        return None
    return ('group', _group_label(conv_group_jobs(form, kind, t, B, g, w, out, ep, False)), share)


def _conv(kind, dtype, t, B, g, w, out, ep):
    plan = conv_form(kind, dtype, t, g, w, out, ep)
    form, x3, _ = plan
    if PROFILE is None and form == 'direct3x3':
        L.check(L.load().sedt_conv3x3_c64(_p(t), _p(w), int(kind == 'dgrad'), _p(ep.get('scale')), _p(ep.get('bias')),
                                          1 if ep.get('act', 0) == ACT_RELU else 0, _p(ep.get('mask')), _p(out), B, g.Hi, g.Wi, 64,
                                          L.stream_ptr()), 'conv3x3_c64')
    elif PROFILE is None and form != 'gemm':
        jobs = conv_group_jobs(form, kind, t, B, g, w, out, ep, x3)
        L.check(L.load().sedt_igemm_group((L.SedtIgemm * len(jobs))(*jobs), len(jobs), BF16, L.stream_ptr()),
                'igemm_group_s2' if form == 's2_parity' else 'igemm_group_dil')
    else:
        dgrad = kind == 'dgrad'
        if L.LAUNCH_LOG is not None and dgrad and not g.plain:
            L.LAUNCH_LOG['conv_dgrad_gather:k%ds%d' % (g.KH, g.sh)] += 1
        M, N, K = (B * g.Hi * g.Wi, g.Ci, g.taps * g.Co) if dgrad else (B * g.Ho * g.Wo, g.Co, g.taps * g.Ci)
        hint = conv_hint(kind, plan, t, B, g, w, out, ep) if PROFILE is not None else None
        if dgrad:
            ep = dict(ep, transposed=0 if g.plain else 1)
        igemm(dtype, M, N, K, t, t.stride(0), w, K, out, out.stride(0), conv=None if g.plain else _geom_tuple(g, dgrad), hint=hint, **ep)
    return out


def conv_fwd(dtype, x, B, g, wf, out=None, **ep):
    if out is None:
        out = torch.empty((B * g.Ho * g.Wo, g.Co), device=x.device, dtype=TORCH_DTYPE[dtype])
    return _conv('fwd', dtype, x, B, g, wf, out, ep)


def conv_dgrad(dtype, dy, B, g, wb, out=None, **ep):
    if out is None:
        out = torch.empty((B * g.Hi * g.Wi, g.Ci), device=dy.device, dtype=TORCH_DTYPE[dtype])
    return _conv('dgrad', dtype, dy, B, g, wb, out, ep)


PROJ_COMPACT = _dev_env('SEDT_PROJ_COMPACT', '1') != '0'


def proj_compact_ok(g):
    return PROJ_COMPACT and g.KH == 1 and g.KW == 1 and (g.sh > 1 or g.sw > 1) and g.ph == 0 and g.pw == 0 and g.dh == 1 and g.dw == 1


def proj_dgrad(dtype, dy, B, g, wb):
    if not proj_compact_ok(g):
        side = conv_dgrad(dtype, dy, B, g, wb)
        return side, dict(ldr=side.stride(0))
    M = B * g.Ho * g.Wo
    side = torch.empty((M, g.Ci), device=dy.device, dtype=TORCH_DTYPE[dtype])
    if L.LAUNCH_LOG is not None:
        L.LAUNCH_LOG['proj_dgrad:%dx%dx%d' % (M, g.Ci, g.Co)] += 1
    igemm(dtype, M, g.Ci, g.Co, dy, dy.stride(0), wb, g.Co, side, side.stride(0))
    return side, dict(ldr=side.stride(0), res_map=(g.Hi, g.Wi, g.sh, g.sw))


def _fused_bias_ok(dtype, dy, x, g):
    return (dtype == BF16 and L.load() is not None and g.Co % 8 == 0 and (g.taps * g.Ci) % 8 == 0 and dy.stride(0) % 8 == 0
            and x.stride(0) % 8 == 0 and dy.data_ptr() % 16 == 0 and x.data_ptr() % 16 == 0 and g.Ci % 8 == 0)


class ReduceBatch(object):

    def __init__(self, shared=False):
        self.jobs, self.keep, self.deferred, self.operands = [], [], [], []
        self.group, self.group_dtype = [], None
        self.shared = shared
        self.expect = []

    def add_gemm(self, dtype, args, shape, code=None):
        self.group.append((args, shape, L.gemm_dtype(dtype) if code is None else code))
        self.group_dtype = dtype

    def _launch_group(self):
        if not self.group:
            return
        lib = L.load()
        if PROFILE is not None:
            for a, shape, code in self.group:
                L.check(lib.sedt_igemm(C.byref(a), code, L.stream_ptr()), 'sedt_igemm')
                PROFILE.append((a, code, shape, (list(self.keep), list(self.operands)), 'wgrad_group'))
        else:
            i = 0
            while i < len(self.group):
                j = i
                while j < len(self.group) and self.group[j][2] == self.group[i][2]:
                    j += 1
                arr = (L.SedtIgemm * (j - i))(*[g[0] for g in self.group[i:j]])
                L.check(lib.sedt_wgrad_group(arr, j - i, self.group[i][2], L.stream_ptr()), 'wgrad_group')
                i = j
        self.group = []

    def defer(self, body, operands):
        self.deferred.append(body)
        self.operands.extend(t for t in operands if t is not None)

    def add(self, slab, sk, R, taps, Ci, rowscale, out, cs, bias_out, cs_splitk=0):
        j = L.SedtReduceJob()
        j.slab, j.out, j.splitk, j.R, j.taps, j.Ci = slab.data_ptr(), out.data_ptr(), sk, R, taps, Ci
        j.cs_splitk = cs_splitk
        j.rowscale = rowscale.data_ptr() if rowscale is not None else None
        j.colsum_slab = cs.data_ptr() if cs is not None else None
        j.bias_out = bias_out.data_ptr() if (cs is not None and bias_out is not None) else None
        self.jobs.append(j)
        self.keep.append((slab, cs, rowscale, None, None) if self.shared else (slab, cs, rowscale, out, bias_out))
        if len(self.jobs) == L.MAX_REDUCE_JOBS and not _co['on'] and not self.shared:
            self._launch_group()
            self._launch()

    def add_colsum(self, partial, nrows, ncols, out):
        j = L.SedtReduceJob()
        j.colsum_slab, j.bias_out, j.splitk, j.R, j.taps, j.Ci = partial.data_ptr(), out.data_ptr(), nrows, ncols, 1, 0
        self.jobs.append(j)
        self.keep.append((partial, None, None, None if self.shared else out, None))

    def _launch(self):
        for i in range(0, len(self.jobs), L.MAX_REDUCE_JOBS):
            chunk = self.jobs[i:i + L.MAX_REDUCE_JOBS]
            arr = (L.SedtReduceJob * len(chunk))(*chunk)
            pf = None
            if self.prefetch is not None and RED_PREFETCH and i + L.MAX_REDUCE_JOBS >= len(self.jobs):
                pf = L.prefetch_arg(self.prefetch)
            L.check(L.load().sedt_multi_wgrad_reduce(arr, len(chunk), pf, L.stream_ptr()), 'multi_wgrad_reduce')
        self.jobs, self.keep = [], []

    prefetch = None

    def collect(self):
        for body in self.deferred:
            body()
        self.deferred = []

    def flush(self, prefetch=None):
        from . import runtime
        self.prefetch = prefetch
        if _co['on'] and not runtime.async_wgrad_on():
            for body in self.deferred:
                body()
            self.deferred = []
            if self.group_dtype in (None, BF16):
                POOL.push(self.group, BF16, self.jobs, [k[:3] for k in self.keep], self.operands)
                self.group, self.jobs, self.keep, self.operands = [], [], [], []
                return
        if self.deferred:
            with runtime.side(*self.operands):
                for body in self.deferred:
                    body()
                self._launch_group()
                self._launch()
            self.deferred, self.operands = [], []
        else:
            self._launch_group()
            self._launch()


DEFER_LAYER_WGRADS = _dev_env('SEDT_DEFER_LAYER_WGRADS', '1') != '0'
_defer = {'on': False}


class defer_layer_wgrads(object):

    def __init__(self, enable=True):
        self.enable = bool(enable) and DEFER_LAYER_WGRADS

    def __enter__(self):
        self.prev = _defer['on']
        _defer['on'] = self.enable
        return self

    def __exit__(self, *exc):
        _defer['on'] = self.prev
        return False


class WgradShare(object):

    def __init__(self):
        self.rb = None
        self.mark = 0

    @staticmethod
    def make():
        return WgradShare() if (_defer['on'] and not _co['on']) else None

    def batch(self):
        if self.rb is None:
            self.rb = ReduceBatch(shared=True)
        return self.rb

    def layer_done(self, last, prefetch=None):
        rb = self.rb
        if rb is None:
            return
        rb.collect()
        if last:
            for param, ptr in rb.expect[:self.mark]:
                g = param.grad
                if g is not None and g.data_ptr() != ptr:
                    raise RuntimeError('a deferred weight gradient was cloned or accumulated by autograd before it was written: '
                                       'defer_layer_wgrads needs parameters whose .grad is None when the backward starts')
            rb.expect = []
            rb.flush(prefetch=prefetch)
            self.rb, self.mark = None, 0
        else:
            self.mark = len(rb.expect)


GRAD_SINK = None


class grad_sink(object):

    def __init__(self, views):
        self.views = dict(views) if views else None

    def __enter__(self):
        global GRAD_SINK
        self.prev, GRAD_SINK = GRAD_SINK, self.views
        return self

    def __exit__(self, *a):
        global GRAD_SINK
        GRAD_SINK = self.prev
        return False


def _sink(param, shape):
    if GRAD_SINK is None or param is None:
        return None
    v = GRAD_SINK.pop(param.data_ptr(), None)
    return v.view(shape) if v is not None and v.numel() == int(np.prod(shape)) else None


def _x3_wgrad_ok(dy, x, g, B):
    if not X3_FAST or dy.dtype != torch.float32 or x.dtype != torch.float32:
        return False
    Co, Ci = g.Co, g.Ci
    if Co % 8 or Ci % 8 or dy.stride(0) % 4 or x.stride(0) % 4 or dy.data_ptr() % 16 or x.data_ptr() % 16:
        return False
    if not g.plain and ((64 % g.Wo) != 0 or g.Ho * g.Wo < 64 or g.Ho < 64 // g.Wo):
        return False
    return B * g.Ho * g.Wo * 3 * Co * 2 < (1 << 31) and B * g.Hi * g.Wi * 3 * Ci * 2 < (1 << 31)


def wgrad(dtype, dy, x, B, g, rowscale=None, out=None, bias_out=None, batch=None, param=None):
    from . import runtime
    lib = L.load()
    Mo, No, Kp = g.Co, g.taps * g.Ci, B * g.Ho * g.Wo
    sk = lib.sedt_igemm_splitk(Mo, No, Kp, dtype)
    own_out = False
    if out is None:
        out = _sink(param, (g.Co, g.Ci, g.KH, g.KW))
        if out is None:
            out = torch.empty((g.Co, g.Ci, g.KH, g.KW), device=dy.device, dtype=torch.float32)
            own_out = True

    def body():
        conv = None if g.plain else _geom_tuple(g)
        if dtype == F32 and L.GEMM_X3 and _x3_wgrad_ok(dy, x, g, B):
            sk3 = max(1, lib.sedt_igemm_splitk(2 * Mo, No, Kp, BF16))
            rows_x = B * g.Hi * g.Wi
            dy3, x3 = _split3([(dy, 0, Kp, Mo, dy.stride(0), 0), (x, 0, rows_x, g.Ci, x.stride(0), 0)])
            slab = torch.empty((3 * sk3, Mo, No), device=dy.device, dtype=torch.float32)
            cs = torch.empty((2 * sk3, Mo), device=dy.device, dtype=torch.float32) if bias_out is not None else None
            a1 = igemm_args(2 * Mo, No, Kp, dy3, 2 * Mo, x3, 2 * g.Ci, slab, No, trans=1, conv=conv, out_f32=1, splitk=sk3, slab=slab,
                            colsum_out=cs)
            x3lo, slab2 = x3[:, g.Ci:2 * g.Ci], slab[2 * sk3:]
            a2 = igemm_args(Mo, No, Kp, dy3, 2 * Mo, x3lo, 2 * g.Ci, slab2, No, trans=1, conv=conv, out_f32=1, splitk=sk3, slab=slab2)
            tb = batch if batch is not None else ReduceBatch()
            tb.add_gemm(dtype, a1, (2 * Mo, No, Kp, 1, 0 if conv is None else 1), code=BF16)
            tb.add_gemm(dtype, a2, (Mo, No, Kp, 1, 0 if conv is None else 1), code=BF16)
            tb.add(slab, 3 * sk3, Mo, g.taps, g.Ci, rowscale, out, cs, bias_out, cs_splitk=2 * sk3)
            tb.keep.append((dy3, x3, None, None, None))
            if batch is None:
                tb._launch_group()
                tb._launch()
            return
        slab = torch.empty((sk, Mo, No), device=dy.device, dtype=torch.float32)
        fused = bias_out is not None and _fused_bias_ok(dtype, dy, x, g)
        cs = torch.empty((sk, Mo), device=dy.device, dtype=torch.float32) if fused else None
        if batch is not None:
            batch.add_gemm(dtype, igemm_args(Mo, No, Kp, dy, dy.stride(0), x, x.stride(0), slab, No, trans=1, conv=conv,
                                             out_f32=1, splitk=sk, slab=slab, colsum_out=cs),
                           (Mo, No, Kp, 1, 0 if conv is None else 1))
            batch.add(slab, sk, Mo, g.taps, g.Ci, rowscale, out, cs, bias_out if fused else None)
        else:
            igemm(dtype, Mo, No, Kp, dy, dy.stride(0), x, x.stride(0), slab, No, trans=1, conv=conv, out_f32=1, splitk=sk,
                  slab=slab, colsum_out=cs)
            L.check(lib.sedt_wgrad_reduce_bias(_p(slab), sk, Mo, g.taps, g.Ci, _p(rowscale), _p(out), _p(cs),
                                               _p(bias_out) if fused else None, L.stream_ptr()), 'wgrad_reduce')
        if bias_out is not None and not fused:
            colsum(dtype, dy, out=bias_out)

    if batch is not None:
        batch.defer(body, (dy, x, rowscale))
        if batch.shared and param is not None and own_out and tuple(param.shape) == tuple(out.shape[:param.dim()]):
            batch.expect.append((param, out.data_ptr()))
    else:
        with runtime.side(dy, x, rowscale):
            body()
    return out


def linear_wgrad(dtype, dy, x, out=None, bias_out=None, batch=None, param=None):
    N, K = dy.shape[1], x.shape[1]
    g = ConvGeom(1, 1, K, N)
    return wgrad(dtype, dy, x, dy.shape[0], g, out=out.view(N, K, 1, 1) if out is not None else None,
                 bias_out=bias_out, batch=batch, param=param).view(N, K)


def colsum(dtype, x, out=None):
    lib = L.load()
    rows, cols = x.shape
    if out is None:
        out = torch.empty((cols,), device=x.device, dtype=torch.float32)
    nb = lib.sedt_colsum_scratch(rows, cols)
    scratch = torch.empty((max(nb // 4, 1),), device=x.device, dtype=torch.float32)
    L.check(lib.sedt_colsum(_p(x), x.stride(0), rows, cols, int(x.dtype == torch.float32), dtype, _p(out), _p(scratch),
                            nb, L.stream_ptr()), 'colsum')
    return out


def dropout_grad(dtype, g, p, seed, seed_ptr=None, out=None):
    rows, cols = g.shape
    if out is None:
        out = torch.empty((rows, cols), device=g.device, dtype=g.dtype)
    L.check(L.load().sedt_dropout_grad(_p(g), g.stride(0), _p(out), out.stride(0), rows, cols, p, seed & 0xffffffff,
                                       _p(seed_ptr), dtype, L.stream_ptr()), 'dropout_grad')
    return out


def add(dtype, a, b, b_mod=0, out=None):
    rows, cols = a.shape
    if out is None:
        out = torch.empty_like(a)
    L.check(L.load().sedt_add(_p(a), _p(b), _p(out), rows, cols, b_mod, dtype, L.stream_ptr()), 'add')
    return out


def add_n(dtype, tensors, out=None):
    _dev_check(*tensors)
    tensors = list(tensors)
    n = len(tensors)
    assert n >= 1 and all(t.shape == tensors[0].shape and t.dtype == TORCH_DTYPE[dtype] and t.is_contiguous() for t in tensors)
    while n > 8:
        tensors = [add_n(dtype, tensors[:8])] + tensors[8:]
        n = len(tensors)
    if out is None:
        out = torch.empty_like(tensors[0])
    arr = (C.c_void_p * n)(*[t.data_ptr() for t in tensors])
    L.check(L.load().sedt_add_n(arr, n, _p(out), tensors[0].numel(), dtype, L.stream_ptr()), 'add_n')
    return out


def cast(x, out_dtype):
    code = {torch.float32: F32, torch.bfloat16: BF16}
    x = x.contiguous()
    out = torch.empty(x.shape, device=x.device, dtype=TORCH_DTYPE[out_dtype])
    L.check(L.load().sedt_cast(_p(x), code[x.dtype], _p(out), out_dtype, x.numel(), L.stream_ptr()), 'cast')
    return out


def relu_mask(dtype, g, y):
    g, y = g.contiguous(), y.contiguous()
    out = torch.empty_like(g)
    L.check(L.load().sedt_relu_mask(_p(g), _p(y), _p(out), g.numel(), dtype, L.stream_ptr()), 'relu_mask')
    return out


def copy2d(jobs):
    for base in range(0, len(jobs), 8):
        chunk = jobs[base:base + 8]
        arr = (L.SedtCopyJob * len(chunk))()
        for n, (sp, dp, outer, inner, ss, ds) in enumerate(chunk):
            arr[n].src, arr[n].dst, arr[n].outer, arr[n].inner, arr[n].src_stride, arr[n].dst_stride = sp, dp, outer, inner, ss, ds
        L.check(L.load().sedt_copy2d(arr, len(chunk), L.stream_ptr()), 'copy2d')


def spsedt_dec_in(dtype, patch, query, B, Q, P, qpp, train, ratio=0.0, keep=None, seed=0, seed_ptr=None):
    D = patch.shape[1]
    assert patch.is_contiguous() and patch.shape[0] == B * P and query.dtype == torch.float32 and query.is_contiguous() and query.shape == (Q, D)
    out = torch.empty((B * Q, D), device=patch.device, dtype=patch.dtype)
    keep_out = torch.empty((Q, B), device=patch.device, dtype=torch.float32) if train else None
    if keep is not None:
        keep = keep.to(device=patch.device, dtype=torch.float32).reshape(Q, B).contiguous()
    L.check(L.load().sedt_spsedt_dec_in(_p(patch), _p(query), _p(keep), _p(keep_out), _p(out), B, Q, P, qpp, D, int(train),
                                        float(ratio), seed & 0xffffffff, _p(seed_ptr), dtype, L.stream_ptr()), 'spsedt_dec_in')
    return out, keep_out


def spsedt_dec_in_bwd(dtype, g, keep, B, Q, P, qpp, train, need_patch=True):
    D = g.shape[1]
    g = g.contiguous()
    d_patch = torch.empty((B * P, D), device=g.device, dtype=g.dtype) if need_patch else None
    d_query = torch.empty((Q, D), device=g.device, dtype=torch.float32)
    L.check(L.load().sedt_spsedt_dec_in_bwd(_p(g), _p(keep), _p(d_patch), _p(d_query), B, Q, P, qpp, D, int(train), dtype, L.stream_ptr()),
            'spsedt_dec_in_bwd')
    return d_patch, d_query


def gelu_fwd(dtype, h, p=0.0, seed=0, seed_ptr=None):
    h = h.contiguous()
    a = torch.empty_like(h)
    L.check(L.load().sedt_gelu_fwd(_p(h), _p(a), h.numel(), p, seed & 0xffffffff, _p(seed_ptr), dtype, L.stream_ptr()), 'gelu_fwd')
    return a


def gelu_bwd(dtype, g, h, p=0.0, seed=0, seed_ptr=None):
    g, h = g.contiguous(), h.contiguous()
    out = torch.empty_like(g)
    L.check(L.load().sedt_gelu_bwd(_p(g), _p(h), _p(out), g.numel(), p, seed & 0xffffffff, _p(seed_ptr), dtype, L.stream_ptr()), 'gelu_bwd')
    return out


def sigmoid_grad(g, s):
    g, s = g.contiguous(), s.contiguous()
    out = torch.empty_like(g)
    L.check(L.load().sedt_sigmoid_grad(_p(g), _p(s), _p(out), g.numel(), L.stream_ptr()), 'sigmoid_grad')
    return out


def layernorm_fwd(dtype, x, gamma, beta, add_t=None, out=None):
    rows, D = x.shape
    assert x.is_contiguous() and (add_t is None or (add_t.is_contiguous() and add_t.shape == x.shape)), 'layernorm_fwd: contiguous rows'
    y2 = torch.empty_like(x) if add_t is not None else None
    if out is not None:
        y, mean, rstd = out
    else:
        y = torch.empty_like(x)
        mean = torch.empty((rows,), device=x.device, dtype=torch.float32)
        rstd = torch.empty_like(mean)
    assert y.is_contiguous() and y.shape == x.shape, 'layernorm_fwd: contiguous rows'
    L.check(L.load().sedt_layernorm_fwd(_p(x), _p(gamma), _p(beta), _p(add_t), _p(y), _p(y2), _p(mean), _p(rstd), rows, D,
                                        dtype, L.stream_ptr()), 'layernorm_fwd')
    return y, y2, mean, rstd


def layernorm_bwd(dtype, dy, x, gamma, mean, rstd, dy2=None, dres=None, want_param_grads=True, batch=None, drop=None, dres2=None):
    lib = L.load()
    rows, D = x.shape
    assert all(t is None or (t.is_contiguous() and t.shape == x.shape) for t in (dy, x, dy2, dres, dres2)), 'layernorm_bwd: contiguous rows'
    dx = torch.empty_like(x)
    dg = torch.empty((D,), device=x.device, dtype=torch.float32) if want_param_grads else None
    db = torch.empty((D,), device=x.device, dtype=torch.float32) if want_param_grads else None
    nb = lib.sedt_layernorm_bwd_scratch(rows, D)
    scratch = torch.empty((nb // 4,), device=x.device, dtype=torch.float32)
    dxd, p_, seed_, sp_ = None, 0.0, 0, None
    if drop is not None and drop[0] > 0:
        p_, seed_, sp_ = drop
        if _dev_env('SEDT_LN_DROP_FUSE', '1') == '0':
            dx, dg, db = layernorm_bwd(dtype, dy, x, gamma, mean, rstd, dy2, dres, want_param_grads, batch, dres2=dres2)
            return dx, dg, db, dropout_grad(dtype, dx, p_, seed_, sp_)
        dxd = torch.empty_like(x)
    deferred = want_param_grads and batch is not None
    L.check(lib.sedt_layernorm_bwd_drop(_p(dy), _p(dy2), _p(x), _p(gamma), _p(mean), _p(rstd), _p(dres), _p(dres2), _p(dx),
                                        None if deferred else _p(dg), None if deferred else _p(db), _p(scratch), nb, rows, D,
                                        _p(dxd), p_, seed_ & 0xffffffff, _p(sp_), dtype, L.stream_ptr()), 'layernorm_bwd')
    if deferred:
        dgb = torch.empty((2 * D,), device=x.device, dtype=torch.float32)
        batch.add_colsum(scratch, nb // (2 * D * 4), 2 * D, dgb)
        dg, db = dgb[:D], dgb[D:]
    if drop is not None:
        return dx, dg, db, (dxd if dxd is not None else dx)
    return dx, dg, db


def attention_instance(dtype, q, k, v, o, Lq, Lk, amask=None, drop_p=0.0, do=None, dq=None, dk=None, dv=None):
    def pl(t):
        return (_p(t), t.stride(0)) if t is not None else (None, 0)
    buf = C.create_string_buffer(96)
    args = pl(q) + pl(k) + pl(v) + pl(o) + pl(do) + pl(dq) + pl(dk) + pl(dv)
    L.load().sedt_attention_describe(*args, int(amask is not None), Lq, Lk, drop_p, dtype, int(do is not None), buf, 96)
    return buf.value.decode()


def attention_fwd(dtype, q, k, v, B, H, Lq, Lk, kpm=None, amask=None, drop_p=0.0, seed=0, seed_ptr=None, out=None):
    if out is None:
        out = torch.empty((B * Lq, H * 32), device=q.device, dtype=q.dtype)
    lse = torch.empty((B, H, Lq), device=q.device, dtype=torch.float32)
    if L.LAUNCH_LOG is not None:
        L.LAUNCH_LOG['attention:' + attention_instance(dtype, q, k, v, out, Lq, Lk, amask, drop_p)] += 1
    L.check(L.load().sedt_attention_fwd(_p(q), q.stride(0), _p(k), k.stride(0), _p(v), v.stride(0), _p(out), out.stride(0),
                                        _p(lse), _p(kpm), _p(amask), B, H, Lq, Lk, drop_p, seed & 0xffffffff, _p(seed_ptr),
                                        dtype, L.stream_ptr()), 'attention_fwd')
    return out, lse


def attention_bwd(dtype, q, k, v, o, do, lse, B, H, Lq, Lk, dq, dk, dv, kpm=None, amask=None, drop_p=0.0, seed=0,
                  seed_ptr=None):
    if L.LAUNCH_LOG is not None:
        L.LAUNCH_LOG['attention:' + attention_instance(dtype, q, k, v, o, Lq, Lk, amask, drop_p, do, dq, dk, dv)] += 1
    L.check(L.load().sedt_attention_bwd(_p(q), q.stride(0), _p(k), k.stride(0), _p(v), v.stride(0), _p(o), o.stride(0),
                                        _p(do), do.stride(0), _p(lse), _p(kpm), _p(amask), _p(dq), dq.stride(0), _p(dk),
                                        dk.stride(0), _p(dv), dv.stride(0), B, H, Lq, Lk, drop_p, seed & 0xffffffff,
                                        _p(seed_ptr), dtype, L.stream_ptr()), 'attention_bwd')
    return dq, dk, dv


NO_RIDE = _dev_env('SEDT_CO_NORIDE', '0') == '1'
CONV3_DIRECT = _dev_env('SEDT_CONV3_DIRECT', '1') != '0'
STEM_DIRECT = _dev_env('SEDT_STEM_DIRECT', '1') != '0'
SLAB_ENC = _dev_env('SEDT_SLAB_ENC', '1') != '0'
SLAB_ENC_BWD = _dev_env('SEDT_SLAB_ENC_BWD', '1') != '0'


SLAB_MIN_WGS = 192
SLAB_MAX_WGS = 320

# ... 849 lines not shown
```

sound_event_detection_transformer_amd/sedt/sedt.py:

```python
import torch
from torch import nn

from .. import functional as Fn
from .. import ops, packing, runtime
from ..ops import ACT_NONE, ACT_RELU, ACT_SIGMOID
from ..utilities.utils import NestedTensor, nested_tensor_from_tensor_list


class HipLinear(nn.Linear):

    def forward(self, x, act=ACT_NONE, out_f32=False):
        lead = x.shape[:-1]
        y = Fn.LinearFn.apply(x.reshape(-1, x.shape[-1]), self.weight, self.bias, act, out_f32, runtime.compute_dtype())
        return y.view(*lead, self.out_features)


class HipConv1x1(nn.Conv2d):

    relu_input = False
    input_bits = None

    def forward(self, x):
        B, C, H, W = x.shape
        tok = x.permute(0, 2, 3, 1).reshape(B * H * W, C)
        bits = self.input_bits() if (self.relu_input and self.input_bits is not None) else None
        if bits is not None and tuple(bits.shape) != (B * H * W, C // 8):
            bits = None
        y = Fn.LinearFn.apply(tok, self.weight.view(self.out_channels, self.in_channels), self.bias, ACT_NONE, False,
                              runtime.compute_dtype(), self.relu_input, bits)
        return y.view(B, H, W, self.out_channels).permute(0, 3, 1, 2)


class MLP(nn.Module):

    def __init__(self, input_dim, hidden_dim, output_dim, num_layers):
        super().__init__()
        self.num_layers = num_layers
        h = [hidden_dim] * (num_layers - 1)
        self.layers = nn.ModuleList(HipLinear(n, k) for n, k in zip([input_dim] + h, h + [output_dim]))

    def forward(self, x, final_act=ACT_NONE, out_f32=False):
        for i, layer in enumerate(self.layers):
            last = i == self.num_layers - 1
            x = layer(x, act=final_act if last else ACT_RELU, out_f32=out_f32 and last)
        return x


class SEDT(nn.Module):

    def __init__(self, backbone, transformer, num_classes, num_queries, aux_loss=False, dec_at=False, pooling=None):
        super().__init__()
        self.pool_mode = None
        if pooling is not None:
            if pooling not in ('max', 'avg', 'attn', 'weighted_sum') or (pooling == 'weighted_sum' and not dec_at):
                raise ValueError(f"pooling={pooling!r}: the reference defines max / avg / attn, and weighted_sum for dec_at models only "
                                 "(sedt.py:47-61, 98-100: without dec_at it fails there with a missing pooling_func)")
            self.pool_mode = pooling
        self.num_queries = num_queries
        self.transformer = transformer
        hidden_dim = transformer.d_model
        self.class_embed = HipLinear(hidden_dim, num_classes + 1)
        self.bbox_embed = MLP(hidden_dim, hidden_dim, 2, 3)
        self.input_proj = HipConv1x1(backbone.num_channels, hidden_dim, kernel_size=1)
        self.backbone = backbone
        body = getattr(backbone[0], 'body', None) if isinstance(backbone, nn.Sequential) else None
        if body is not None and hasattr(body, 'premasked_consumer'):
            self.input_proj.relu_input = True
            self.input_proj.input_bits = lambda: getattr(body, 'out_bits', None)
            body.premasked_consumer = True
        self.aux_loss = aux_loss
        self.dec_at = dec_at
        self.pooling = pooling
        if self.dec_at:
            self.query_embed = nn.Embedding(num_queries + 1, hidden_dim)
            self.weak_class_embed = HipLinear(hidden_dim, num_classes)
        else:
            self.query_embed = nn.Embedding(num_queries, hidden_dim)
        if self.pool_mode == 'attn':
            self.attn_dense_softmax = HipLinear(hidden_dim, num_classes)

    def pack_plan(self):
        dt, dev = runtime.compute_dtype(), self.query_embed.weight.device
        key = (dt, str(dev))
        plans = self.__dict__.setdefault('_plans', {})
        if key not in plans:
            def factory():
                body = self.backbone[0].body
                convs = []
                l34 = set(id(p_) for layer in (body.layer3, body.layer4) for p_ in layer.parameters())
                bn_only = [(body.conv1.weight, body.bn1.tensors())]
                for layer in (body.layer1, body.layer2, body.layer3, body.layer4):
                    for b in layer:
                        convs += [(b.conv1.weight, b.bn1.tensors()), (b.conv2.weight, b.bn2.tensors()), (b.conv3.weight, b.bn3.tensors())]
                        if b.downsample is not None:
                            convs.append((b.downsample[0].weight, b.downsample[1].tensors()))
                lin = [self.input_proj.weight]
                frags = []
                for l in self.transformer.encoder.layers:
                    lin += [l.self_attn.in_proj_weight, l.self_attn.out_proj.weight, l.linear1.weight, l.linear2.weight]
                    frags += [l.self_attn.in_proj_weight, l.self_attn.out_proj.weight, l.linear1.weight, l.linear2.weight]
                for l in self.transformer.decoder.layers:
                    lin += [l.self_attn.in_proj_weight, l.self_attn.out_proj.weight, l.multihead_attn.in_proj_weight,
                            l.multihead_attn.out_proj.weight, l.linear1.weight, l.linear2.weight]
                    frags += [l.self_attn.in_proj_weight, l.self_attn.out_proj.weight, l.multihead_attn.in_proj_weight,
                              l.multihead_attn.out_proj.weight, l.linear1.weight, l.linear2.weight]
                lin += [self.class_embed.weight] + [m.weight for m in self.bbox_embed.layers]
                frags += [m.weight for m in self.bbox_embed.layers[:2]]
                for name in ('weak_class_embed', 'patch2query', 'attn_dense_softmax'):
                    if hasattr(self, name):
                        lin.append(getattr(self, name).weight)
                if hasattr(self, 'feature_align'):
                    lin += [m.weight for m in self.feature_align.layers]
                fus = [(b, ops.BLOCK_FORMS.get(ops.fusable_form(b.cfg))) for layer in (body.layer1, body.layer2, body.layer3, body.layer4)
                       for b in layer]
                cfr = [w for b, row in fus if row and row.nops == 3 for w in (b.conv1.weight, b.conv2.weight, b.conv3.weight)]
                cfr += [w for b, row in fus if row and row.nops == 4
                        for w in (b.conv1.weight, b.conv2.weight, b.conv3.weight, b.downsample[0].weight)]
                if ops.IGEMM_BREG:
                    have = set(id(w) for w in cfr)
                    cfr += [w for w, _ in convs if id(w) not in have and id(w) in l34]
                return packing.PackPlan(dt, dev, convs, lin, bn_only, frags, cfr)
            plans[key] = packing.PlanSet(factory)
        return plans[key]

    def forward(self, samples):
        with self.pack_plan():
            return self._forward(samples)

    def _forward(self, samples):
        if isinstance(samples, (list, torch.Tensor)):
            samples = nested_tensor_from_tensor_list(samples)
        features, pos = self.backbone(samples)
        src, mask = features[-1].decompose()
        assert mask is not None
        out = {}
        hs, memory = self.transformer(self.input_proj(src), mask, self.query_embed.weight, pos[-1], enc_at_embed=None)
        q0 = 1 if self.dec_at else 0
        b = self.bbox_embed.layers
        wa = (self.weak_class_embed.weight, self.weak_class_embed.bias) if self.dec_at else (None, None)
        res = Fn.HeadsFn.apply(hs, self.class_embed.weight, self.class_embed.bias, b[0].weight, b[0].bias, b[1].weight, b[1].bias,
                               b[2].weight, b[2].bias, wa[0], wa[1], runtime.compute_dtype())
        cls_full, box_full = res[0], res[1]
        outputs_class, outputs_coord = cls_full[:, :, q0:, :], box_full[:, :, q0:, :]
        if self.dec_at:
            out['at'] = res[2].squeeze()
        out['pred_logits'] = outputs_class[-1]
        out['pred_boxes'] = outputs_coord[-1]
        if self.pool_mode is not None:
            mode, Q = self.pool_mode, cls_full.shape[2] - q0
            attn = self.attn_dense_softmax(hs[-1][:, q0:, :].contiguous(), out_f32=True) if mode == 'attn' else None
            at_p = Fn.PoolAtFn.apply(cls_full[-1], box_full[-1] if mode == 'weighted_sum' else None, attn, mode, q0, Q)
            out['at_p'] = at_p.squeeze() if mode in ('max', 'avg') else at_p
        if self.aux_loss:
            out['aux_outputs'] = self._set_aux_loss(outputs_class, outputs_coord)
            out['_stacked'] = (cls_full, box_full)
            out['_q0'] = q0
        return out

    def _set_aux_loss(self, outputs_class, outputs_coord):
        return [{'pred_logits': a, 'pred_boxes': b} for a, b in zip(outputs_class[:-1], outputs_coord[:-1])]


import torch.nn.functional as F

from ..utilities import box_ops


class TargetTables(object):

    def __init__(self, batch, ns, n_lab, device, max_targets=32, with_ratio=False, slots=4, dynamic_split=False,
                 weak_mask_none=False):
        if not 1 <= max_targets <= 63:
            raise ValueError('max_targets must be in 1..63 (one wave lane per target)')
        self.dynamic = bool(dynamic_split)
        self.weak_mask_none = bool(weak_mask_none)
        self.B, self.max_targets, self.dev = batch, max_targets, device
        self.ns, self.n_lab = (batch, batch) if self.dynamic else (ns, max(n_lab, ns))
        self.cur_ns, self.cur_n_lab = ns, max(n_lab, ns)
        ns = self.ns
        n_off = batch + ns + 4
        n_lab_e, n_box_e = batch * max_targets, max(ns, 1) * max_targets
        o_lab = (4 * n_off + 7) // 8 * 8
        o_box = o_lab + 8 * n_lab_e
        o_rat = o_box + 8 * n_box_e
        total = o_rat + (4 * n_lab_e if with_ratio else 0)
        self._lay = (n_off, o_lab, n_lab_e, o_box, n_box_e, o_rat, total)
        self._blob = torch.zeros(total, dtype=torch.uint8, device=device)
        self.off = self._blob[:4 * n_off].view(torch.int32)
        self.lab_cat = self._blob[o_lab:o_box].view(torch.int64)
        self.box_cat = self._blob[o_box:o_rat].view(torch.float32).view(n_box_e, 2)
        self.ratio_cat = self._blob[o_rat:total].view(torch.float32) if with_ratio else None
        if with_ratio:
            self.ratio_cat.fill_(1.0)
        self.split = self.off[batch + ns + 2:] if self.dynamic else None
        self._pin = [torch.zeros(total, dtype=torch.uint8).pin_memory() for _ in range(slots)] if device.type == 'cuda' else None
        self._ev = [None] * slots
        self._slot = 0

    def as_dict(self):
        return {'lab_cat': self.lab_cat, 'box_cat': self.box_cat, 'ratio_cat': self.ratio_cat,
                'lab_off': self.off[:self.B + 1], 'box_off': self.off[self.B + 1:self.B + self.ns + 2]}

    @torch.no_grad()
    def load(self, targets, ns=None, n_lab=None):
        import numpy as np
        B = self.B
        if hasattr(targets, 'blob'):
            return self._load_device(targets)
        if len(targets) != B:
            raise ValueError(f'expected {B} clips, got {len(targets)}')
        if ns is not None or n_lab is not None:
            if not self.dynamic:
                if (ns, n_lab) != (self.cur_ns, self.cur_n_lab):
                    raise ValueError('these tables were built for a fixed strong/weak split: TargetTables(dynamic_split=True)')
            else:
                ns = self.cur_ns if ns is None else ns
                self.cur_ns, self.cur_n_lab = ns, max(ns if n_lab is None else n_lab, ns)
                if not 0 <= self.cur_ns <= self.cur_n_lab <= B:
                    raise ValueError(f'split {self.cur_ns} | {self.cur_n_lab} outside 0..{B}')
        ns = self.cur_ns
        nlab = [int(t['labels'].shape[0]) for t in targets]
        nbox = [int(targets[b]['boxes'].reshape(-1, 2).shape[0]) for b in range(ns)]
        if max(nlab + nbox + [0]) > self.max_targets:
            raise ValueError(f'a clip has more than max_targets={self.max_targets} events')
        if any(nb > nl for nb, nl in zip(nbox, nlab)):
            raise ValueError('a strong clip has more boxes than labels')
        if self.ratio_cat is None and any('ratio' in t for t in targets):
            raise ValueError('targets carry pseudo-label ratios: build TargetTables(with_ratio=True)')
        off = [0]
        for n in nlab:
            off.append(off[-1] + n)
        off.append(0)
        for n in nbox:
            off.append(off[-1] + n)
        off += [off[-1]] * (self.ns - ns)
        off += [self.cur_ns, self.cur_n_lab]
        nl, nb = sum(nlab), sum(nbox)
        n_off, o_lab, n_lab_e, o_box, n_box_e, o_rat, total = self._lay
        host = self._pin is not None and all(not t['labels'].is_cuda and not t['boxes'].is_cuda for t in targets)
        if self._pin is None or host:
            k = self._slot
            self._slot = (k + 1) % len(self._ev)
            if self._pin is not None:
                if self._ev[k] is not None:
                    self._ev[k].synchronize()
                buf = self._pin[k].numpy()
            else:
                buf = np.zeros(total, np.uint8)
            buf[:4 * n_off].view(np.int32)[:len(off)] = off
            if nl:
                buf[o_lab:o_lab + 8 * nl].view(np.int64)[:] = torch.cat([t['labels'].reshape(-1) for t in targets]).numpy()
            if nb:
                buf[o_box:o_box + 8 * nb].view(np.float32)[:] = torch.cat([targets[b]['boxes'].reshape(-1, 2).float() for b in range(ns)]).numpy().reshape(-1)
            if self.ratio_cat is not None and nl:
                buf[o_rat:o_rat + 4 * nl].view(np.float32)[:] = np.concatenate(
                    [t['ratio'].detach().float().reshape(-1).cpu().numpy() if 'ratio' in t else np.ones(n, np.float32) for t, n in zip(targets, nlab)])
            if self._pin is not None:
                self._blob.copy_(self._pin[k], non_blocking=True)
                self._ev[k] = torch.cuda.Event()
                self._ev[k].record()
            else:
                self._blob.copy_(torch.from_numpy(buf))
            return self
        k = self._slot
        self._slot = (k + 1) % len(self._ev)
        if self._ev[k] is not None:
            self._ev[k].synchronize()
        pin_off = self._pin[k][:4 * n_off].view(torch.int32)
        pin_off[:len(off)].copy_(torch.tensor(off, dtype=torch.int32))
        self.off.copy_(pin_off, non_blocking=True)
        self._ev[k] = torch.cuda.Event()
        self._ev[k].record()
        if nl:
            self.lab_cat[:nl].copy_(torch.cat([t['labels'].reshape(-1) for t in targets]), non_blocking=True)
        if nb:
            self.box_cat[:nb].copy_(torch.cat([targets[b]['boxes'].reshape(-1, 2).float() for b in range(ns)]), non_blocking=True)
        if self.ratio_cat is not None and nl:
            src = targets[0]['labels'].device
            self.ratio_cat[:nl].copy_(torch.cat([t['ratio'].detach().float().reshape(-1).to(src) if 'ratio' in t else
                                                 torch.ones(n, device=src) for t, n in zip(targets, nlab)]), non_blocking=True)
        return self


    def _load_device(self, targets):
        if self.dynamic:
            raise NotImplementedError('targets built on the device cannot be copied into dynamic-split tables (mix-up): the merged batch '
                                      'is planned from them on the device by load_mixed(); load() is for static-split tables')
        B, M = self.B, self.max_targets
        Bs = int(targets.B)
        ns_src, n_lab_src = min(int(getattr(targets, 'ns', Bs)), B), min(int(getattr(targets, 'n_lab', Bs)), B)
        if Bs < B or (ns_src, n_lab_src) != (self.ns, self.n_lab) or targets.max_targets != M:
            raise ValueError(f'targets built on the device are {ns_src} strong | {n_lab_src} labelled of {Bs} clips of up to '
                             f'{targets.max_targets} events; these tables hold {self.ns} strong | {self.n_lab} labelled of {B} clips, '
                             f'max_targets={M}')
        src = targets.blob
        if src.numel() != 8 * Bs + 16 + 16 * Bs * M or src.device != self._blob.device:
            raise ValueError('targets built on the device: the blob does not have this table layout')
        n_off, o_lab, n_lab_e, o_box, n_box_e, o_rat, total = self._lay
        if Bs == B and self.ns == B:
            self._blob[:o_rat].copy_(src, non_blocking=True)
        else:
            ns = self.ns
            so_lab = 8 * Bs + 16
            so_box = so_lab + 8 * Bs * M
            self._blob[:4 * (B + 1)].copy_(src[:4 * (B + 1)], non_blocking=True)
            self._blob[o_lab:o_lab + 8 * B * M].copy_(src[so_lab:so_lab + 8 * B * M], non_blocking=True)
            self._blob[4 * (B + 1):4 * (B + ns + 2)].copy_(src[4 * (Bs + 1):4 * (Bs + ns + 2)], non_blocking=True)
            if ns:
                self._blob[o_box:o_box + 8 * ns * M].copy_(src[so_box:so_box + 8 * ns * M], non_blocking=True)
        if self.ratio_cat is not None:
            self.ratio_cat.fill_(1.0)
        return self

    @torch.no_grad()
    def load_mixed(self, targets, lam, index, mix_num, max_events, jobs, status=None):
        import numpy as np
        from .. import ops
        from ..utilities.mixup import lam_pair
        from ..utilities.transforms import PinnedRing
        if not self.dynamic or self.ratio_cat is None:
            raise ValueError('load_mixed fills dynamic-split tables with ratio: TargetTables(dynamic_split=True, with_ratio=True)')
        if not hasattr(targets, 'blob'):
            raise ValueError('load_mixed takes targets built on the device (DeviceTargets); plan host lists with plan_mixup_data and load()')
        B, Bs = self.B, int(targets.B)
        if Bs < B:
            raise ValueError(f'expected at least {B} clips, got {Bs}')
        ns, n_lab = min(int(targets.ns), B), min(int(targets.n_lab), B)
        index = np.ascontiguousarray(index, np.int32).reshape(-1)
        if index.shape[0] != B or (B and (index.min() < 0 or index.max() >= B)):
            raise ValueError(f'load_mixed: index holds one partner in 0..{B - 1} per clip')
        if not 0 <= int(mix_num) <= ns:
            raise ValueError(f'load_mixed: mix-up of the first {mix_num} clips needs as many strong clips, the batch has {ns}: the '
                             'reference then mixes weak clips as well, which this route does not plan')
        if not 1 <= int(max_events) <= self.max_targets:
            raise ValueError(f'load_mixed: max_events={max_events} outside 1..max_targets={self.max_targets}')
        if self.dev.type != 'cuda' or targets.blob.device != self._blob.device:
            raise RuntimeError('load_mixed runs on the device (the HIP path has no CPU fallback)')
        if getattr(self, '_ring', None) is None:
            self._ring = PinnedRing(self.dev)
            self.plan_status = torch.zeros(B, dtype=torch.int32, device=self.dev)
        raw = self._ring.upload(np.concatenate([lam_pair(lam).view(np.uint8), index.view(np.uint8)]))
        d_lam, d_index = raw[:8].view(torch.float32), raw[8:8 + 4 * B].view(torch.int32)
        ops.mixup_plan(targets.blob, Bs, targets.max_targets, B, ns, n_lab, d_index, d_lam, int(mix_num), int(max_events),
                       self.max_targets, self._blob, jobs, self.plan_status if status is None else status)
        return self


ALPHA_FL, GAMMA_FL = 0.5, 1.0


class _CriterionFn(torch.autograd.Function):

    @staticmethod
    def forward(ctx, logits_all, boxes_all, at, dense, empty_weight, layer_of, w_ce, w_bbox, w_giou, w_weak, fl, nonfinite, q0,
                at_p=None, w_weak_p=0.0):
        from .. import ops
        ctx.set_materialize_grads(False)
        f32c = lambda t: t.detach() if (t.dtype == torch.float32 and t.is_contiguous()) else t.detach().float().contiguous()
        out, total, ctx.state = ops.set_criterion(f32c(logits_all), f32c(boxes_all), None if at is None else f32c(at), dense,
                                                  empty_weight, layer_of, w_ce, w_bbox, w_giou, w_weak, fl=fl, alpha_fl=ALPHA_FL,
                                                  gamma_fl=GAMMA_FL, nonfinite=nonfinite, q0=q0,
                                                  at_p=None if at_p is None else f32c(at_p), w_weak_p=w_weak_p,
                                                  wp_all=bool(dense.get('wp_all', False)))
        ctx.dts = (logits_all.dtype, boxes_all.dtype, None if at is None else at.dtype, None if at_p is None else at_p.dtype)
        return out, total

    @staticmethod
    def backward(ctx, g, gtotal):
        from .. import ops
        if g is None and gtotal is None:
            return (None,) * 15
        gl, gb, gat, gat_p = ops.set_criterion_bwd(ctx.state, g, gtotal)
        return (gl.to(ctx.dts[0]), gb.to(ctx.dts[1]), None if gat is None else gat.to(ctx.dts[2]),
                None, None, None, None, None, None, None, None, None, None,
                None if gat_p is None else gat_p.to(ctx.dts[3]), None)


class _FeatureLossFn(torch.autograd.Function):

    @staticmethod
    def forward(ctx, pred_all, gt, dense, layer_of, num_boxes, wvec, nonfinite=None, base_total=None):
        from .. import ops
        ctx.set_materialize_grads(False)
        res = ops.feature_loss(pred_all.detach().float().contiguous(), gt.detach().float().contiguous(), dense,
                               layer_of, num_boxes, wvec, nonfinite, None if base_total is None else base_total.detach().float())
        out, ctx.dpred = res[0], res[1]
        ctx.wvec, ctx.dt = wvec, pred_all.dtype
        inv = [0] * len(layer_of)
        for d, ml in enumerate(layer_of):
            inv[ml] = d
        ctx.inv = inv
        ctx.has_base = base_total is not None
        return (out, res[2]) if ctx.has_base else out

    @staticmethod
    def backward(ctx, g, gtotal=None):
        from .. import ops
        if g is None and gtotal is None:
            return (None,) * 8
        L = len(ctx.inv)
        gl = gt_ = None
        if g is not None:
            g = g.contiguous().float()
            gl, gt_ = g[:L], g[L:]
        if gtotal is not None:
            gtotal = gtotal.reshape(1).float()
            gt_ = gtotal if gt_ is None else gt_ + gtotal
        d = ops.scale_layers(ctx.dpred, gl, gt_, ctx.wvec, ctx.inv)
        ctx.dpred = None
        return d.to(ctx.dt), None, None, None, None, None, None, (gtotal.reshape(()) if (ctx.has_base and gtotal is not None) else None)


class SetCriterion(nn.Module):

    def __init__(self, num_classes, matcher, weight_dict, eos_coef, losses):
        super().__init__()
        self.num_classes, self.matcher, self.weight_dict = num_classes, matcher, weight_dict
        self.eos_coef, self.losses = eos_coef, losses
        empty_weight = torch.ones(self.num_classes + 1)
        empty_weight[-1] = self.eos_coef
        self.register_buffer('empty_weight', empty_weight)
        self.last_total = None
        self._wvec = {}
        self.nonfinite = None
        self.host_compute = None

    @torch.no_grad()
    def prepare(self, outputs, targets, weak_mask=None, strong_mask=None, normalize=False, fine_tune=False, fl=False,
                ft_rand=None):
        import numpy as np
        from .. import lib as L_
        if strong_mask is None or strong_mask.start not in (None, 0) or strong_mask.step not in (None, 1):
            raise NotImplementedError('strong_mask must be slice(0, n): strongly labelled clips come first in every driver')
        layers = [outputs] + list(outputs.get('aux_outputs', []))
        L = len(layers)
        dev = outputs['pred_logits'].device
        ns = len(targets[strong_mask])
        st = targets[:ns]
        logits = torch.stack([o['pred_logits'][:ns] for o in layers]).detach().float()
        boxes = torch.stack([o['pred_boxes'][:ns] for o in layers]).detach().float()
        Q = logits.shape[2]
        sizes = [int(len(t['boxes'])) for t in st]
        Nt = sum(sizes)
        n_lab = (weak_mask.stop if weak_mask is not None else strong_mask.stop) if 'at' in outputs else ns
# ... 248 lines not shown
```

sound_event_detection_transformer_amd/sedt/transformer.py:

```python
import copy
from typing import Optional

import torch
from torch import nn, Tensor

from .. import functional as Fn
from .. import runtime


def _tokens(x):
    B, C, H, W = x.shape
    return x.permute(0, 2, 3, 1).reshape(B * H * W, C)


def _u8(mask):
    return None if mask is None else mask.contiguous().view(torch.uint8)


def _activation_name(activation):
    if activation in ("relu", "gelu"):
        return activation
    if activation == "glu":
        raise ValueError('activation "glu" halves the FFN width: linear2 of the reference layer (transformer.py:160) fails on it too')
    raise RuntimeError(F"activation should be relu/gelu, not {activation}.")


class TransformerEncoderLayer(nn.Module):
    def __init__(self, d_model, nhead, dim_feedforward=2048, dropout=0.1, activation="relu", normalize_before=False):
        super().__init__()
        self.activation = _activation_name(activation)
        self.self_attn = nn.MultiheadAttention(d_model, nhead, dropout=dropout)
        self.linear1 = nn.Linear(d_model, dim_feedforward)
        self.dropout = nn.Dropout(dropout)
        self.linear2 = nn.Linear(dim_feedforward, d_model)
        self.norm1 = nn.LayerNorm(d_model)
        self.norm2 = nn.LayerNorm(d_model)
        self.dropout1 = nn.Dropout(dropout)
        self.dropout2 = nn.Dropout(dropout)
        self.normalize_before = normalize_before
        self.nhead, self.p = nhead, dropout

    def params(self):
        a = self.self_attn
        return (a.in_proj_weight, a.in_proj_bias, a.out_proj.weight, a.out_proj.bias, self.linear1.weight,
                self.linear1.bias, self.linear2.weight, self.linear2.bias, self.norm1.weight, self.norm1.bias,
                self.norm2.weight, self.norm2.bias)

    def forward_tokens(self, x, pos, kpm, B, S, src_mask=None, chain=None, wg_share=None, layer_idx=0):
        cfg = dict(dt=runtime.compute_dtype(), B=B, S=S, H=self.nhead, dropout=self.p, training=self.training,
                   pre_norm=self.normalize_before, chain=chain, act=self.activation, wg_share=wg_share, layer_idx=layer_idx)
        return Fn.EncoderLayerFn.apply(x, pos, kpm, src_mask, cfg, *self.params())

    def forward(self, src, src_mask: Optional[Tensor] = None, src_key_padding_mask: Optional[Tensor] = None,
                pos: Optional[Tensor] = None):
        S, B, d = src.shape
        x = src.transpose(0, 1).reshape(B * S, d)
        p = (pos if pos is not None else torch.zeros_like(src)).transpose(0, 1).reshape(B * S, d)
        y = self.forward_tokens(x, p, _u8(src_key_padding_mask), B, S, src_mask)
        return y.view(B, S, d).transpose(0, 1)


class TransformerDecoderLayer(nn.Module):
    def __init__(self, d_model, nhead, dim_feedforward=2048, dropout=0.1, activation="relu", normalize_before=False):
        super().__init__()
        self.activation = _activation_name(activation)
        self.self_attn = nn.MultiheadAttention(d_model, nhead, dropout=dropout)
        self.multihead_attn = nn.MultiheadAttention(d_model, nhead, dropout=dropout)
        self.linear1 = nn.Linear(d_model, dim_feedforward)
        self.dropout = nn.Dropout(dropout)
        self.linear2 = nn.Linear(dim_feedforward, d_model)
        self.norm1 = nn.LayerNorm(d_model)
        self.norm2 = nn.LayerNorm(d_model)
        self.norm3 = nn.LayerNorm(d_model)
        self.dropout1 = nn.Dropout(dropout)
        self.dropout2 = nn.Dropout(dropout)
        self.dropout3 = nn.Dropout(dropout)
        self.normalize_before = normalize_before
        self.nhead, self.p = nhead, dropout

    def params(self):
        a, c = self.self_attn, self.multihead_attn
        return (a.in_proj_weight, a.in_proj_bias, a.out_proj.weight, a.out_proj.bias,
                c.in_proj_weight, c.in_proj_bias, c.out_proj.weight, c.out_proj.bias,
                self.linear1.weight, self.linear1.bias, self.linear2.weight, self.linear2.bias,
                self.norm1.weight, self.norm1.bias, self.norm2.weight, self.norm2.bias, self.norm3.weight, self.norm3.bias)

    def forward_tokens(self, tgt, mem, mem_pos, qpos, kpm, B, S, Q, tgt_mask=None, kv_fused=False, out=None, acc=None, share=None,
                       layer_idx=0, chain=None, wg_share=None):
        cfg = dict(kv_fused=kv_fused, dt=runtime.compute_dtype(), B=B, S=S, Q=Q, H=self.nhead, dropout=self.p, training=self.training,
                   pre_norm=self.normalize_before, out=out, acc_mem=None if acc is None else acc[0],
                   acc_qpos=None if acc is None else acc[1], share=share, layer_idx=layer_idx, chain=chain, act=self.activation,
                   wg_share=wg_share)
        return Fn.DecoderLayerFn.apply(tgt, mem, mem_pos, qpos, kpm, tgt_mask, cfg, *self.params())


def _get_clones(module, N):
    return nn.ModuleList([copy.deepcopy(module) for _ in range(N)])


class TransformerEncoder(nn.Module):
    def __init__(self, encoder_layer, num_layers, norm=None):
        super().__init__()
        self.layers = _get_clones(encoder_layer, num_layers)
        self.num_layers = num_layers
        self.norm = norm

    def forward_tokens(self, x, pos, kpm, B, S, chain=None):
        from .. import ops
        wg = ops.WgradShare.make() if (torch.is_grad_enabled() and len(self.layers) > 1
                                       and all(p.requires_grad for l in self.layers for p in l.parameters())) else None
        for li, layer in enumerate(self.layers):
            x = layer.forward_tokens(x, pos, kpm, B, S, chain=chain, wg_share=wg, layer_idx=li)
        if self.norm is not None:
            x = Fn.LayerNormFn.apply(x, self.norm.weight, self.norm.bias, runtime.compute_dtype())
        return x


class TransformerDecoder(nn.Module):
    def __init__(self, decoder_layer, num_layers, norm=None, return_intermediate=False):
        super().__init__()
        self.layers = _get_clones(decoder_layer, num_layers)
        self.num_layers = num_layers
        self.norm = norm
        self.return_intermediate = return_intermediate

    def forward_tokens(self, tgt, mem, pos, qpos, kpm, B, S, Q, tgt_mask=None, chain=None):
        dt = runtime.compute_dtype()
        mem_pos = Fn.AddFn.apply(mem, pos, 0, dt)
        qpos = Fn.CastFn.apply(qpos, dt)
        out = tgt
        outs = []
        R, d, n = tgt.shape[0], tgt.shape[1], len(self.layers)
        stack = (torch.empty((n * R, d), device=tgt.device, dtype=runtime.torch_dtype())
                 if (self.return_intermediate and n > 1 and all(l.normalize_before for l in self.layers)) else None)
        acc = ((Fn.GradAccumulator(n), Fn.GradAccumulator(n)) if (torch.is_grad_enabled() and all(l.normalize_before for l in self.layers)
                                                                  and not pos.requires_grad) else None)
        share = {} if (stack is not None and acc is not None) else None
        from .. import ops
        wg = ops.WgradShare.make() if (torch.is_grad_enabled() and n > 1 and all(p.requires_grad for l in self.layers for p in l.parameters())) else None
        for li, layer in enumerate(self.layers):
            out = layer.forward_tokens(out, mem, mem_pos, qpos, kpm, B, S, Q, tgt_mask, kv_fused=not pos.requires_grad,
                                       out=None if stack is None else stack[li * R:(li + 1) * R], acc=acc, share=share, layer_idx=li,
                                       chain=chain, wg_share=wg)
            outs.append(out)
        if self.return_intermediate:
            stacked = Fn.StackViewFn.apply(stack, share, *outs) if stack is not None else (torch.cat(outs) if n > 1 else outs[0])
            return Fn.LayerNormFn.apply(stacked, self.norm.weight, self.norm.bias, dt).view(n, B, Q, d)
        return Fn.LayerNormFn.apply(out, self.norm.weight, self.norm.bias, dt).view(1, B, Q, d)


class Transformer(nn.Module):
    def __init__(self, d_model=512, nhead=8, num_encoder_layers=6, num_decoder_layers=6, dim_feedforward=2048,
                 dropout=0.1, activation="relu", normalize_before=False, return_intermediate_dec=False, self_sup=False):
        super().__init__()
        if d_model // nhead != 32 or d_model % nhead:
            raise ValueError('the HIP attention kernels implement head dim 32 (d_model / nhead)')
        enc_layer = TransformerEncoderLayer(d_model, nhead, dim_feedforward, dropout, activation, normalize_before)
        enc_norm = nn.LayerNorm(d_model) if normalize_before else None
        self.encoder = TransformerEncoder(enc_layer, num_encoder_layers, enc_norm)
        dec_layer = TransformerDecoderLayer(d_model, nhead, dim_feedforward, dropout, activation, normalize_before)
        self.decoder = TransformerDecoder(dec_layer, num_decoder_layers, nn.LayerNorm(d_model),
                                          return_intermediate=return_intermediate_dec)
        self._reset_parameters()
        self.d_model, self.nhead, self.self_sup = d_model, nhead, self_sup

    def _reset_parameters(self):
        for p in self.parameters():
            if p.dim() > 1:
                nn.init.xavier_uniform_(p)

    def _zero_tokens(self, rows, cols, device):
        key = (rows, cols, runtime.torch_dtype(), str(device))
        z = self.__dict__.setdefault('_zeros', {}).get(key)
        if z is not None:
            from ..utilities.utils import pin_if_capturing
            return pin_if_capturing(z)
        if z is None:
            z = torch.zeros((rows, cols), device=device, dtype=runtime.torch_dtype())
            if not (z.is_cuda and torch.cuda.is_current_stream_capturing()):
                if len(self._zeros) > 8:
                    self._zeros.clear()
                self._zeros[key] = z
        return z

    def forward(self, src, mask, query_embed, pos_embed, enc_at_embed=None, decoder_mask=None):
        if enc_at_embed is not None:
            raise NotImplementedError('enc_at_embed is unreachable from SEDT.forward (sedt.py:88) and not built')
        if not src.is_cuda:
            raise RuntimeError('the SEDT transformer runs on the MI355X HIP path only (no CPU fallback)')
        dt = runtime.compute_dtype()
        B, C, H, W = src.shape
        S = H * W
        x = _tokens(src)
        pos = _tokens(pos_embed)
        kpm = _u8(mask.flatten(1))
        tgt = None
        if self.self_sup:
            Q = query_embed.shape[0]
            qpos = query_embed.permute(1, 0, 2).reshape(B * Q, C)
        else:
            Q = query_embed.shape[0]
            tgt = self._zero_tokens(B * Q, C, src.device)
            qpos = Fn.BroadcastRowsFn.apply(query_embed, tgt, B, dt)
        if tgt is None:
            tgt = self._zero_tokens(B * Q, C, src.device)
        from .. import ops
        chain = ops.BackwardChain()
        memory = self.encoder.forward_tokens(x, pos, kpm, B, S, chain=chain)
        self.cut_memory = memory if getattr(self, 'keep_cut', False) else None
        tmask = decoder_mask.float().contiguous() if (self.self_sup and decoder_mask is not None) else None
        hs = self.decoder.forward_tokens(tgt, memory, pos, qpos, kpm, B, S, Q, tmask, chain=chain)
        if self.self_sup:
            return hs, memory.view(B, H, W, C).permute(0, 3, 1, 2)
        return hs, memory.view(B, S, C)


def build_transformer(args):
    return Transformer(d_model=args.hidden_dim, dropout=args.dropout, nhead=args.nheads,
                       dim_feedforward=args.dim_feedforward, num_encoder_layers=args.enc_layers,
                       num_decoder_layers=args.dec_layers, normalize_before=args.pre_norm,
                       return_intermediate_dec=True, self_sup=args.self_sup)
```

Before: 12880 clips/s.

## Join lone weight-gradient reductions into shared batches and multi-unit reduce blocks

Result: no change. 12950 clips/s (median of 6 runs) (+0.6%).

```diff
diff --git a/sound_event_detection_transformer_amd/csrc/misc.hip b/sound_event_detection_transformer_amd/csrc/misc.hip
--- a/sound_event_detection_transformer_amd/csrc/misc.hip
+++ b/sound_event_detection_transformer_amd/csrc/misc.hip
@@ -34,6 +34,8 @@
   const uint32_t* pf[3]; int pf_lines[3];
 };
 
+constexpr int RED_UNITS = 4;
+constexpr int RED_BATCH = 8;
 __host__ __device__ inline int reduce_job_mode(const SedtReduceJob& J) {
   if ((reinterpret_cast<uintptr_t>(J.slab) | reinterpret_cast<uintptr_t>(J.out)) & 15) return 2;
   if (J.taps == 1 && (J.Ci & 3) == 0) return J.splitk >= 16 ? 3 : 0;
@@ -44,18 +46,33 @@
   const long per = (long)J.R * J.taps * J.Ci;
   const int mode = reduce_job_mode(J);
   if (mode == 0) return (int)((per + 1023) / 1024);
-  if (mode == 1) return J.R * (J.Ci / 64);
+  if (mode == 1) return (J.R * (J.Ci / 64) + RED_UNITS - 1) / RED_UNITS;
   return (int)((per + 255) / 256);
 }
 
+__device__ __forceinline__ void acc4(float4& s, const float4& a) { s.x += a.x; s.y += a.y; s.z += a.z; s.w += a.w; }
+
+template <int NB>
+__device__ __forceinline__ void red_strided(const float* sp, long per, int z, int splitk, float4& s0, float4& s1) {
+  for (; z < splitk; z += 4 * NB) {
+    float4 a[NB];
+#pragma unroll
+    for (int i = 0; i < NB; ++i)
+      if (z + 4 * i < splitk) a[i] = *reinterpret_cast<const float4*>(sp + (long)(z + 4 * i) * per);
+#pragma unroll
+    for (int i = 0; i < NB; ++i)
+      if (z + 4 * i < splitk) { if (i & 1) acc4(s1, a[i]); else acc4(s0, a[i]); }
+  }
+}
+
 __global__ __launch_bounds__(256) void multi_wgrad_reduce_kernel(const ReduceJobs jobs) {
-  __shared__ float tile[9][65];
+  __shared__ float tile[RED_UNITS][9][65];
   if (blockIdx.x < 256 && jobs.pf_lines[0] + jobs.pf_lines[1] + jobs.pf_lines[2] > 0) {
     const int slot = blockIdx.x >> 3, nslots = min(32, max(1, (int)(gridDim.x >> 3)));
     uint32_t acc = 0;
     for (int r = 0; r < 3; ++r)
       for (int j = slot * 256 + threadIdx.x; j < jobs.pf_lines[r]; j += nslots * 256) acc ^= jobs.pf[r][(long)j * 32];
-    if (acc == 0x9e3779b9u && jobs.n < 0) tile[0][0] = 1.f;
+    if (acc == 0x9e3779b9u && jobs.n < 0) tile[0][0][0] = 1.f;
   }
   int lo = 0, hi = jobs.n - 1;
   while (lo < hi) {
@@ -95,17 +112,7 @@
     float4 s0 = make_float4(0.f, 0.f, 0.f, 0.f), s1 = s0;
     if (e < per) {
       const float* sp = J.slab + e;
-      int z = zg;
-      for (; z + 4 < J.splitk; z += 8) {
-        const float4 a = *reinterpret_cast<const float4*>(sp + (long)z * per);
-        const float4 b = *reinterpret_cast<const float4*>(sp + (long)(z + 4) * per);
-        s0.x += a.x; s0.y += a.y; s0.z += a.z; s0.w += a.w;
-        s1.x += b.x; s1.y += b.y; s1.z += b.z; s1.w += b.w;
-      }
-      if (z < J.splitk) {
-        const float4 a = *reinterpret_cast<const float4*>(sp + (long)z * per);
-        s0.x += a.x; s0.y += a.y; s0.z += a.z; s0.w += a.w;
-      }
+      red_strided<RED_BATCH>(sp, per, zg, J.splitk, s0, s1);
     }
     zsum[zg][q] = make_float4(s0.x + s1.x, s0.y + s1.y, s0.z + s1.z, s0.w + s1.w);
     __syncthreads();
@@ -146,45 +153,70 @@
     }
     *reinterpret_cast<float4*>(J.out + e) = s;
   } else if (mode == 1) {
-    const int chunks = J.Ci / 64;
-    const int r = blk / chunks, c0 = (blk - r * chunks) * 64;
-    if (r >= J.R) return;
-    const int n = J.taps * 64;
-    const float sc = J.rowscale ? J.rowscale[r] : 1.f;
-    const long rbase = (long)r * J.taps * J.Ci;
-    for (int i = threadIdx.x; i < n / 4; i += 256) {
-      const int tap = i >> 4, c = (i & 15) * 4;
-      const float* sp = J.slab + rbase + (long)tap * J.Ci + c0 + c;
-      float4 v = *reinterpret_cast<const float4*>(sp), u = make_float4(0.f, 0.f, 0.f, 0.f);
-      int z = 1;
-      for (; z + 2 <= J.splitk; z += 2) {
-        const float4 a = *reinterpret_cast<const float4*>(sp + (long)z * per);
-        const float4 b = *reinterpret_cast<const float4*>(sp + (long)(z + 1) * per);
-        v.x += a.x; v.y += a.y; v.z += a.z; v.w += a.w;
-        u.x += b.x; u.y += b.y; u.z += b.z; u.w += b.w;
+    const int chunks = J.Ci / 64, units = J.R * chunks;
+    const int ul = threadIdx.x >> 6, u_ = blk * RED_UNITS + ul;
+    const int c = (threadIdx.x & 15) * 4, tg = (threadIdx.x >> 4) & 3;
+    if (u_ < units) {
+      const int r = u_ / chunks, c0 = (u_ - r * chunks) * 64;
+      const float sc = J.rowscale ? J.rowscale[r] : 1.f;
+      const float* sp = J.slab + (long)r * J.taps * J.Ci + c0 + c;
+      if (J.splitk <= 2) {
+        float4 a[3][2];
+#pragma unroll
+        for (int k = 0; k < 3; ++k)
+#pragma unroll
+          for (int i = 0; i < 2; ++i)
+            if (tg + 4 * k < J.taps && i < J.splitk) a[k][i] = *reinterpret_cast<const float4*>(sp + (long)(tg + 4 * k) * J.Ci + (long)i * per);
+#pragma unroll
+        for (int k = 0; k < 3; ++k)
+          if (tg + 4 * k < J.taps) {
+            float4 v = a[k][0];
+            if (1 < J.splitk) acc4(v, a[k][1]);
+            float* tp = &tile[ul][tg + 4 * k][c];
+            tp[0] = (v.x + 0.f) * sc; tp[1] = (v.y + 0.f) * sc; tp[2] = (v.z + 0.f) * sc; tp[3] = (v.w + 0.f) * sc;
+          }
+      } else {
+#pragma unroll
+        for (int k = 0; k < 3; ++k)
+          if (tg + 4 * k < J.taps) {
+            const float* tp = sp + (long)(tg + 4 * k) * J.Ci;
+            float4 v, u = make_float4(0.f, 0.f, 0.f, 0.f);
+            for (int z = 0; z < J.splitk; z += RED_BATCH) {
+              float4 a[RED_BATCH];
+#pragma unroll
+              for (int i = 0; i < RED_BATCH; ++i)
+                if (z + i < J.splitk) a[i] = *reinterpret_cast<const float4*>(tp + (long)(z + i) * per);
+#pragma unroll
+              for (int i = 0; i < RED_BATCH; ++i)
+                if (z + i < J.splitk) {
+                  if (i == 0 && z == 0) v = a[0];
+                  else if (i & 1) acc4(v, a[i]);
+                  else acc4(u, a[i]);
+                }
+            }
+            float* o = &tile[ul][tg + 4 * k][c];
+            o[0] = (v.x + u.x) * sc; o[1] = (v.y + u.y) * sc; o[2] = (v.z + u.z) * sc; o[3] = (v.w + u.w) * sc;
+          }
       }
-      if (z < J.splitk) {
-        const float4 a = *reinterpret_cast<const float4*>(sp + (long)z * per);
-        v.x += a.x; v.y += a.y; v.z += a.z; v.w += a.w;
-      }
-      tile[tap][c] = (v.x + u.x) * sc; tile[tap][c + 1] = (v.y + u.y) * sc;
-      tile[tap][c + 2] = (v.z + u.z) * sc; tile[tap][c + 3] = (v.w + u.w) * sc;
     }
     __syncthreads();
-    float* o = J.out + ((long)r * J.Ci + c0) * J.taps;
+    const int nu = min(RED_UNITS, units - blk * RED_UNITS), n = J.taps * 64;
+    float* o = J.out + (long)blk * RED_UNITS * n;
     if (J.taps == 9) {
-      for (int i = threadIdx.x; i < n / 4; i += 256) {
+      for (int i = threadIdx.x; i < nu * (n / 4); i += 256) {
+        const int un = i / 144, i4 = 4 * (i - un * 144);
         float4 q;
-        { const int k = 4 * i, c = k / 9, tap = k - c * 9; q.x = tile[tap][c]; }
-        { const int k = 4 * i + 1, c = k / 9, tap = k - c * 9; q.y = tile[tap][c]; }
-        { const int k = 4 * i + 2, c = k / 9, tap = k - c * 9; q.z = tile[tap][c]; }
-        { const int k = 4 * i + 3, c = k / 9, tap = k - c * 9; q.w = tile[tap][c]; }
+        { const int k = i4, cc = k / 9, tap = k - cc * 9; q.x = tile[un][tap][cc]; }
+        { const int k = i4 + 1, cc = k / 9, tap = k - cc * 9; q.y = tile[un][tap][cc]; }
+        { const int k = i4 + 2, cc = k / 9, tap = k - cc * 9; q.z = tile[un][tap][cc]; }
+        { const int k = i4 + 3, cc = k / 9, tap = k - cc * 9; q.w = tile[un][tap][cc]; }
         *reinterpret_cast<float4*>(o + 4 * i) = q;
       }
     } else {
-      for (int i = threadIdx.x; i < n; i += 256) {
-        const int c = i / J.taps, tap = i - c * J.taps;
-        o[i] = tile[tap][c];
+      for (int i = threadIdx.x; i < nu * n; i += 256) {
+        const int un = i / n, k = i - un * n;
+        const int cc = k / J.taps, tap = k - cc * J.taps;
+        o[i] = tile[un][tap][cc];
       }
     }
   } else {
diff --git a/sound_event_detection_transformer_amd/functional.py b/sound_event_detection_transformer_amd/functional.py
--- a/sound_event_detection_transformer_amd/functional.py
+++ b/sound_event_detection_transformer_amd/functional.py
@@ -45,14 +45,16 @@
 class LinearFn(Function):
 
     @staticmethod
-    def forward(ctx, x, weight, bias, act, out_f32, dt, relu_input=False, x_bits=None):
+    def forward(ctx, x, weight, bias, act, out_f32, dt, relu_input=False, x_bits=None, wg_share=None):
         x = _as(x, dt)
+        ctx.wg_share = wg_share
         ctx.relu_input = relu_input
         ctx.x_bits = x_bits if relu_input else None
         ctx.dt, ctx.act, ctx.out_f32 = dt, act, out_f32
         ctx.has_bias = bias is not None
         ctx.skinny = ops.skinny_ok(weight.shape[0], weight.shape[1]) and out_f32 and weight.is_contiguous()
         if ctx.skinny:
+            assert wg_share is None
             y = ops.skinny_linear_fwd(dt, x, weight, bias, act, True)
             ctx.save_for_backward(x, weight, y if act != ACT_NONE else None)
             return y
@@ -70,7 +72,7 @@
             gx, gw, gb = ops.skinny_linear_bwd(dt, gy.float() if gy.dtype != torch.float32 else gy, y, weight, x, ctx.act,
                                                mask=x if ctx.relu_input else None, need_gx=ctx.needs_input_grad[0],
                                                need_gw=ctx.needs_input_grad[1], need_gb=ctx.has_bias and ctx.needs_input_grad[2])
-            return gx, gw, gb, None, None, None, None, None
+            return gx, gw, gb, None, None, None, None, None, None
         if ctx.act == ACT_SIGMOID:
             gy = ops.sigmoid_grad(gy.float() if gy.dtype != torch.float32 else gy, y.float() if y.dtype != torch.float32 else y)
         elif ctx.act == ACT_RELU:
@@ -83,13 +85,18 @@
             else:
                 gx = ops.linear(dt, g, ctx.wb, mask=x, ldm=x.stride(0)) if ctx.relu_input else ops.linear(dt, g, ctx.wb)
         gb = torch.empty((g.shape[1],), device=g.device, dtype=torch.float32) if (ctx.has_bias and ctx.needs_input_grad[2]) else None
-        if ctx.needs_input_grad[1]:
+        share = ctx.wg_share
+        if share is not None:
+            ctx.wg_share = None
+            gw = ops.linear_wgrad(dt, g, x, bias_out=gb, batch=share.batch())
+            share.layer_done(last=True)
+        elif ctx.needs_input_grad[1]:
             gw = ops.linear_wgrad(dt, g, x, bias_out=gb)
         else:
             gw = None
             if gb is not None:
                 ops.colsum(dt, g, out=gb)
-        return gx, gw, gb, None, None, None, None, None
+        return gx, gw, gb, None, None, None, None, None, None
 
 
 class PoolAtFn(Function):
@@ -117,11 +124,13 @@
 class HeadsFn(Function):
 
     @staticmethod
-    def forward(ctx, hs, wc, bc, w1, b1, w2, b2, w3, b3, wa, ba, dt):
+    def forward(ctx, hs, wc, bc, w1, b1, w2, b2, w3, b3, wa, ba, dt, wg_share=None):
         Lh, B, Qp, d = hs.shape
         x = _as(hs, dt).view(Lh * B * Qp, d)
         tr = any(ctx.needs_input_grad)
         ctx.slab = None
+        ctx.wg_share = wg_share if (ops.JOIN_LONE_WGRADS and ctx.needs_input_grad[0]) else None
+        ctx.leafs = (wc, bc, w1, b1, w2, b2, w3, b3, wa, ba) if ctx.wg_share is not None else None
         if ops.heads_slab_ok(dt, d, wc.shape[0], 0 if wa is None else wa.shape[0], hs.numel() // d) and wc.is_contiguous() and w3.is_contiguous():
             fr = [packing.lookup_frag(w) for w in (w1, w2)]
             if all(f is not None for f in fr):
@@ -160,7 +169,8 @@
             w1t, w2t = ctx.slab
             dhs, g_h1, g_h2, part = ops.heads_bwd(x, h1, h2, box.view(M, 2), at, f32c(g_cls).view(M, -1), f32c(g_box).view(M, 2),
                                                   f32c(g_at) if ctx.has_at else None, wc, w3, wa, w2t, w1t, Lh, B, Qp)
-            rb = ops.ReduceBatch()
+            share = ctx.wg_share
+            rb = share.batch() if share is not None else ops.ReduceBatch()
             d_b2 = torch.empty((d,), device=x.device, dtype=torch.float32)
             d_w2 = ops.linear_wgrad(dt, g_h2, h1, bias_out=d_b2, batch=rb)
             d_b1 = torch.empty((d,), device=x.device, dtype=torch.float32)
@@ -168,17 +178,19 @@
             NG = C1 + CA + 2
             tot = torch.empty((NG * 257,), device=x.device, dtype=torch.float32)
             rb.add_colsum(part, part.shape[0], NG * 257, tot)
-            rb.flush()
             tw, tb = tot[:NG * 256].view(NG, 256), tot[NG * 256:]
             d_wc, d_bc = tw[:C1], tb[:C1]
             d_w3, d_b3 = tw[C1 + CA:], tb[C1 + CA:]
             d_wa = d_ba = None
             if ctx.has_at:
                 d_wa, d_ba = tw[C1:C1 + CA], tb[C1:C1 + CA]
-            return (dhs.view(Lh, B, Qp, d), d_wc, d_bc, d_w1, d_b1, d_w2, d_b2, d_w3, d_b3, d_wa, d_ba, None)
+            grads = (d_wc, d_bc, d_w1, d_b1, d_w2, d_b2, d_w3, d_b3, d_wa, d_ba)
+            _heads_wgrads_out(ctx, rb, grads)
+            return (dhs.view(Lh, B, Qp, d),) + grads + (None, None)
         w1b, w2b = ctx.wb
         f32 = lambda t: t.contiguous() if t.dtype == torch.float32 else t.contiguous().float()
-        rb = ops.ReduceBatch()
+        share = ctx.wg_share
+        rb = share.batch() if share is not None else ops.ReduceBatch()
         dhs, d_wc, d_bc = ops.skinny_linear_bwd(dt, f32(g_cls).view(M, -1), None, wc, x, ACT_NONE, batch=rb)
         g_h2, d_w3, d_b3 = ops.skinny_linear_bwd(dt, f32(g_box).view(M, 2), box.view(M, 2), w3, h2, ACT_SIGMOID, mask=h2, batch=rb)
         d_b2 = torch.empty((g_h2.shape[1],), device=x.device, dtype=torch.float32)
@@ -196,8 +208,20 @@
                 ga = f32(g_at).view(B, -1)
                 _, d_wa, d_ba = ops.skinny_linear_bwd(dt, ga, at.view(B, -1), wa, xa, ACT_SIGMOID,
                                                       gx_acc=dhs.view(Lh, B, Qp, d)[Lh - 1, :, 0, :], batch=rb)
+        grads = (d_wc, d_bc, d_w1, d_b1, d_w2, d_b2, d_w3, d_b3, d_wa, d_ba)
+        _heads_wgrads_out(ctx, rb, grads)
+        return (dhs.view(Lh, B, Qp, d),) + grads + (None, None)
+
+
+def _heads_wgrads_out(ctx, rb, grads):
+    share, leafs = ctx.wg_share, ctx.leafs
+    ctx.wg_share = ctx.leafs = None
+    if share is None:
         rb.flush()
-        return (dhs.view(Lh, B, Qp, d), d_wc, d_bc, d_w1, d_b1, d_w2, d_b2, d_w3, d_b3, d_wa, d_ba, None)
+        return
+    for p_, g_ in zip(leafs, grads):
+        rb.expect_grad(p_, g_)
+    share.layer_done(last=False)
 
 
 class SplitClipsFn(Function):
@@ -568,7 +592,8 @@
         (w_in, b_in, w_o, b_o, w1, b1, w2, b2, g1, be1, g2, be2) = P
         gx2 = _as(gx2, dt)
         share = cfg.get('wg_share') if not (sv.get('slab') is not None and ops.SLAB_ENC_BWD) else None
-        rb = share.batch() if share is not None else ops.ReduceBatch()
+        tail = cfg.get('wg_tail') if share is None else None
+        rb = share.batch() if share is not None else (tail.batch() if tail is not None else ops.ReduceBatch())
         if sv.get('slab') is not None and ops.SLAB_ENC_BWD:
             B, S, H = cfg['B'], cfg['S'], cfg['H']
             wint, wot, w1t, w2t = sv['slab']
@@ -600,9 +625,13 @@
             gx, part1 = ops.encoder_qkv_bwd(dqk, dv, sv['x'], sv['m1'], sv['r1'], g1, gx1, wint, B, S)
             dgb1 = torch.empty((2 * E,), device=dev, dtype=torch.float32)
             rb.add_colsum(part1, part1.shape[0], 2 * E, dgb1)
-            rb.flush(prefetch=sv.get('bwd_next'))
+            grads = (d_win, d_bin, d_wo, d_bo, d_w1, d_b1, d_w2, d_b2, dgb1[:E], dgb1[E:], dgb2[:E], dgb2[E:])
+            if tail is not None:
+                _leave_to_tail(tail, rb, P, grads)
+            else:
+                rb.flush(prefetch=sv.get('bwd_next'))
             ctx.sv = None
-            return (gx, None, None, None, None, d_win, d_bin, d_wo, d_bo, d_w1, d_b1, d_w2, d_b2, dgb1[:E], dgb1[E:], dgb2[:E], dgb2[E:])
+            return (gx, None, None, None, None) + grads
         if cfg['pre_norm']:
             g_x1n, d_w1, d_b1, d_w2, d_b2 = _ffn_bwd(dt, sv['ffn'], gx2, w1, w2, batch=rb)
             gx1, d_g2, d_be2, gx1d = ops.layernorm_bwd(dt, g_x1n, sv['x1'], g2, sv['m2'], sv['r2'], dres=gx2, batch=rb,
@@ -618,12 +647,21 @@
                                                        drop=_drop_args(sv['mha'], dev))
             g_qk, _, g_v, d_win, d_bin, d_wo, d_bo = _mha_bwd(dt, sv['mha'], g_t, w_in, w_o, batch=rb, g_dropped=g_td)
             gx = ops.add(dt, ops.add(dt, g_qk, g_v), g_t)
+        grads = (d_win, d_bin, d_wo, d_bo, d_w1, d_b1, d_w2, d_b2, d_g1, d_be1, d_g2, d_be2)
         if share is not None:
             share.layer_done(last=cfg.get('layer_idx', 0) == 0)
+        elif tail is not None:
+            _leave_to_tail(tail, rb, P, grads)
         else:
             rb.flush()
         ctx.sv = None
-        return (gx, None, None, None, None, d_win, d_bin, d_wo, d_bo, d_w1, d_b1, d_w2, d_b2, d_g1, d_be1, d_g2, d_be2)
+        return (gx, None, None, None, None) + grads
+
+
+def _leave_to_tail(tail, rb, params, grads):
+    for p_, g_ in zip(params, grads):
+        rb.expect_grad(p_, g_)
+    tail.layer_done(last=False)
 
 
 class DecoderLayerFn(Function):
diff --git a/sound_event_detection_transformer_amd/ops.py b/sound_event_detection_transformer_amd/ops.py
--- a/sound_event_detection_transformer_amd/ops.py
+++ b/sound_event_detection_transformer_amd/ops.py
@@ -654,6 +654,10 @@
 
     prefetch = None
 
+    def expect_grad(self, param, grad):
+        if param is not None and grad is not None:
+            self.expect.append((param, grad.data_ptr()))
+
     def collect(self):
         for body in self.deferred:
             body()
@@ -683,6 +687,7 @@
 
 
 DEFER_LAYER_WGRADS = _dev_env('SEDT_DEFER_LAYER_WGRADS', '1') != '0'
+JOIN_LONE_WGRADS = _dev_env('SEDT_JOIN_LONE_WGRADS', '1') != '0'
 _defer = {'on': False}
 
 
@@ -722,16 +727,20 @@
             return
         rb.collect()
         if last:
-            for param, ptr in rb.expect[:self.mark]:
-                g = param.grad
-                if g is not None and g.data_ptr() != ptr:
-                    raise RuntimeError('a deferred weight gradient was cloned or accumulated by autograd before it was written: '
-                                       'defer_layer_wgrads needs parameters whose .grad is None when the backward starts')
-            rb.expect = []
+            self._check()
             rb.flush(prefetch=prefetch)
             self.rb, self.mark = None, 0
         else:
             self.mark = len(rb.expect)
+
+    def _check(self):
+        rb = self.rb
+        for param, ptr in rb.expect[:self.mark]:
+            g = param.grad
+            if g is not None and g.data_ptr() != ptr:
+                raise RuntimeError('a deferred weight gradient was cloned or accumulated by autograd before it was written: '
+                                   'defer_layer_wgrads needs parameters whose .grad is None when the backward starts')
+        rb.expect = []
 
 
 GRAD_SINK = None
diff --git a/sound_event_detection_transformer_amd/sedt/sedt.py b/sound_event_detection_transformer_amd/sedt/sedt.py
--- a/sound_event_detection_transformer_amd/sedt/sedt.py
+++ b/sound_event_detection_transformer_amd/sedt/sedt.py
@@ -20,14 +20,14 @@
     relu_input = False
     input_bits = None
 
-    def forward(self, x):
+    def forward(self, x, wg_share=None):
         B, C, H, W = x.shape
         tok = x.permute(0, 2, 3, 1).reshape(B * H * W, C)
         bits = self.input_bits() if (self.relu_input and self.input_bits is not None) else None
         if bits is not None and tuple(bits.shape) != (B * H * W, C // 8):
             bits = None
         y = Fn.LinearFn.apply(tok, self.weight.view(self.out_channels, self.in_channels), self.bias, ACT_NONE, False,
-                              runtime.compute_dtype(), self.relu_input, bits)
+                              runtime.compute_dtype(), self.relu_input, bits, wg_share)
         return y.view(B, H, W, self.out_channels).permute(0, 3, 1, 2)
 
 
@@ -102,8 +102,6 @@
                 for l in self.transformer.decoder.layers:
                     lin += [l.self_attn.in_proj_weight, l.self_attn.out_proj.weight, l.multihead_attn.in_proj_weight,
                             l.multihead_attn.out_proj.weight, l.linear1.weight, l.linear2.weight]
-                    frags += [l.self_attn.in_proj_weight, l.self_attn.out_proj.weight, l.multihead_attn.in_proj_weight,
-                              l.multihead_attn.out_proj.weight, l.linear1.weight, l.linear2.weight]
                 lin += [self.class_embed.weight] + [m.weight for m in self.bbox_embed.layers]
                 frags += [m.weight for m in self.bbox_embed.layers[:2]]
                 for name in ('weak_class_embed', 'patch2query', 'attn_dense_softmax'):
@@ -134,12 +132,16 @@
         src, mask = features[-1].decompose()
         assert mask is not None
         out = {}
-        hs, memory = self.transformer(self.input_proj(src), mask, self.query_embed.weight, pos[-1], enc_at_embed=None)
+        tail = ops.WgradShare.make() if (ops.JOIN_LONE_WGRADS and torch.is_grad_enabled() and self.input_proj.weight.requires_grad) else None
+        hs, memory = self.transformer(self.input_proj(src, wg_share=tail), mask, self.query_embed.weight, pos[-1], enc_at_embed=None,
+                                      wg_tail=tail)
         q0 = 1 if self.dec_at else 0
         b = self.bbox_embed.layers
         wa = (self.weak_class_embed.weight, self.weak_class_embed.bias) if self.dec_at else (None, None)
+        dec = self.transformer.decoder
+        wg, dec.wg_share = getattr(dec, 'wg_share', None), None
         res = Fn.HeadsFn.apply(hs, self.class_embed.weight, self.class_embed.bias, b[0].weight, b[0].bias, b[1].weight, b[1].bias,
-                               b[2].weight, b[2].bias, wa[0], wa[1], runtime.compute_dtype())
+                               b[2].weight, b[2].bias, wa[0], wa[1], runtime.compute_dtype(), wg)
         cls_full, box_full = res[0], res[1]
         outputs_class, outputs_coord = cls_full[:, :, q0:, :], box_full[:, :, q0:, :]
         if self.dec_at:
diff --git a/sound_event_detection_transformer_amd/sedt/transformer.py b/sound_event_detection_transformer_amd/sedt/transformer.py
--- a/sound_event_detection_transformer_amd/sedt/transformer.py
+++ b/sound_event_detection_transformer_amd/sedt/transformer.py
@@ -46,9 +46,10 @@
                 self.linear1.bias, self.linear2.weight, self.linear2.bias, self.norm1.weight, self.norm1.bias,
                 self.norm2.weight, self.norm2.bias)
 
-    def forward_tokens(self, x, pos, kpm, B, S, src_mask=None, chain=None, wg_share=None, layer_idx=0):
+    def forward_tokens(self, x, pos, kpm, B, S, src_mask=None, chain=None, wg_share=None, layer_idx=0, wg_tail=None):
         cfg = dict(dt=runtime.compute_dtype(), B=B, S=S, H=self.nhead, dropout=self.p, training=self.training,
-                   pre_norm=self.normalize_before, chain=chain, act=self.activation, wg_share=wg_share, layer_idx=layer_idx)
+                   pre_norm=self.normalize_before, chain=chain, act=self.activation, wg_share=wg_share, layer_idx=layer_idx,
+                   wg_tail=wg_tail if all(p.requires_grad for p in self.params()) else None)
         return Fn.EncoderLayerFn.apply(x, pos, kpm, src_mask, cfg, *self.params())
 
     def forward(self, src, src_mask: Optional[Tensor] = None, src_key_padding_mask: Optional[Tensor] = None,
@@ -105,12 +106,12 @@
         self.num_layers = num_layers
         self.norm = norm
 
-    def forward_tokens(self, x, pos, kpm, B, S, chain=None):
+    def forward_tokens(self, x, pos, kpm, B, S, chain=None, wg_tail=None):
         from .. import ops
         wg = ops.WgradShare.make() if (torch.is_grad_enabled() and len(self.layers) > 1
                                        and all(p.requires_grad for l in self.layers for p in l.parameters())) else None
         for li, layer in enumerate(self.layers):
-            x = layer.forward_tokens(x, pos, kpm, B, S, chain=chain, wg_share=wg, layer_idx=li)
+            x = layer.forward_tokens(x, pos, kpm, B, S, chain=chain, wg_share=wg, layer_idx=li, wg_tail=wg_tail if li == 0 else None)
         if self.norm is not None:
             x = Fn.LayerNormFn.apply(x, self.norm.weight, self.norm.bias, runtime.compute_dtype())
         return x
@@ -138,6 +139,7 @@
         share = {} if (stack is not None and acc is not None) else None
         from .. import ops
         wg = ops.WgradShare.make() if (torch.is_grad_enabled() and n > 1 and all(p.requires_grad for l in self.layers for p in l.parameters())) else None
+        self.wg_share = wg if ops.JOIN_LONE_WGRADS else None
         for li, layer in enumerate(self.layers):
             out = layer.forward_tokens(out, mem, mem_pos, qpos, kpm, B, S, Q, tgt_mask, kv_fused=not pos.requires_grad,
                                        out=None if stack is None else stack[li * R:(li + 1) * R], acc=acc, share=share, layer_idx=li,
@@ -183,7 +185,7 @@
                 self._zeros[key] = z
         return z
 
-    def forward(self, src, mask, query_embed, pos_embed, enc_at_embed=None, decoder_mask=None):
+    def forward(self, src, mask, query_embed, pos_embed, enc_at_embed=None, decoder_mask=None, wg_tail=None):
         if enc_at_embed is not None:
             raise NotImplementedError('enc_at_embed is unreachable from SEDT.forward (sedt.py:88) and not built')
         if not src.is_cuda:
@@ -206,7 +208,7 @@
             tgt = self._zero_tokens(B * Q, C, src.device)
         from .. import ops
         chain = ops.BackwardChain()
-        memory = self.encoder.forward_tokens(x, pos, kpm, B, S, chain=chain)
+        memory = self.encoder.forward_tokens(x, pos, kpm, B, S, chain=chain, wg_tail=wg_tail)
         self.cut_memory = memory if getattr(self, 'keep_cut', False) else None
         tmask = decoder_mask.float().contiguous() if (self.self_sup and decoder_mask is not None) else None
         hs = self.decoder.forward_tokens(tgt, memory, pos, qpos, kpm, B, S, Q, tmask, chain=chain)
```
